# eivindeb/fixed-wing-gym

Measured on AMD Instinct MI355X. Metric: env-steps/sec, higher is better.
Workload: dtype f32

## Files before the change

fixed-wing-gym_amd/csrc/fwgym.hip:

```cpp
#include <math.h>
#include <stdio.h>
#include <string.h>
#include <string>
#include <vector>
#include "fwgym_env.h"
#include "fwgym_actor.h"
#include "fwgym_learner.h"

__device__ __forceinline__ float wave_sum(float v) { return wave_sum64(v); }

struct SpecWords { unsigned w[sizeof(DevCfg) / 4]; };
static_assert(sizeof(SpecWords) == sizeof(DevCfg), "DevCfg must be made of 32-bit members only");
#if defined(FWG_SPECS_FILE)
#include FWG_SPECS_FILE
#elif defined(FWG_WITH_SPECS)
#include "generated/specs.inc"
#else
#define FWG_SPEC_LIST(X)
#endif
#ifndef FWG_SHAPE_LIST
#define FWG_SHAPE_LIST(X)
#endif
#define FWG_SHAPE_BASE FWG_INSTANCE_SHAPE
#define FWG_DEFINE_SPEC(i) static constexpr DevCfg kSpec##i = __builtin_bit_cast(DevCfg, kSpecWords##i);
FWG_SPEC_LIST(FWG_DEFINE_SPEC)
template <int SPEC> struct SpecCfg {
    static constexpr int obs_dim = 16;
    static constexpr bool rollout_ok = false;
    static constexpr bool one_rk4_step = false;
    static __device__ __forceinline__ const DevCfg& get(const DevCfg* cp) { return *cp; }
};
#define FWG_SPEC_GETTER(i)                                                                                \
    template <> struct SpecCfg<i> {                                                                       \
        static constexpr int obs_dim = kSpec##i.obs_dim;                                                  \
        static constexpr bool one_rk4_step = kSpec##i.nsub == 1;                                          \
         \
        static constexpr bool rollout_ok = kSpec##i.obs_log == 0 && kSpec##i.obs_dim <= 64;               \
        static __device__ __forceinline__ const DevCfg& get(const DevCfg*) { return kSpec##i; }           \
    };
FWG_SPEC_LIST(FWG_SPEC_GETTER)
#define FWG_SHAPE_OBJECT(i) static constexpr DevCfg kShape##i = as_shape(kSpec##i);
FWG_SHAPE_LIST(FWG_SHAPE_OBJECT)
#define FWG_SHAPE_GETTER(i)                                                                               \
    template <> struct SpecCfg<FWG_SHAPE_BASE + i> {                                                      \
        static constexpr int obs_dim = kSpec##i.obs_dim;                                                  \
        static constexpr bool one_rk4_step = kSpec##i.nsub == 1;                                          \
        static constexpr bool rollout_ok = false;    \
        static __device__ __forceinline__ const DevCfg& get(const DevCfg*) { return kShape##i; }          \
    };
FWG_SHAPE_LIST(FWG_SHAPE_GETTER)

template <int SPEC> struct KernelTypes {
    typedef LdsTable Tab;
    typedef LdsTable Obs;
    static constexpr bool generic = true;
    static __device__ __forceinline__ Tab tab(float* lds, const LdsMap& M, int lane) { return Tab{lds + M.tab + lane}; }
    static __device__ __forceinline__ Obs obs(float* lds, const LdsMap& M, int lane) { return Obs{lds + M.obs + lane}; }
};
#define FWG_SPEC_TYPES(i)                                                                                     \
    template <> struct KernelTypes<i> {                      \
        typedef RegTable<FWG_TAB_ROWS> Tab;                                                                   \
        typedef RegTable<kSpec##i.obs_dim> Obs;                                                               \
        static constexpr bool generic = false;                                                                \
        static __device__ __forceinline__ Tab tab(float*, const LdsMap&, int) { return Tab(); }               \
        static __device__ __forceinline__ Obs obs(float*, const LdsMap&, int) { return Obs(); }               \
    };
FWG_SPEC_LIST(FWG_SPEC_TYPES)
#define FWG_SHAPE_TYPES(i) template <> struct KernelTypes<FWG_SHAPE_BASE + i> : KernelTypes<i> {};
FWG_SHAPE_LIST(FWG_SHAPE_TYPES)

struct NoHeadStats { static constexpr bool enabled = false; const float* mean = nullptr; float ret_mean = 0.f; unsigned ctr = 0u; };
struct HeadStats { static constexpr bool enabled = true; const float* mean; float ret_mean; unsigned ctr; };
template <class OB, class HS = NoHeadStats>
__device__ __forceinline__ void step_moments(const DevCfg& c, const KArgs& A, const OB& ob, float reward, bool done, bool valid,
                                             int lane, long e, int sub, float ret_prev, const HS& hs = HS()) {
#ifndef FWG_ABL_NO_ACC
    const int D = c.obs_dim;
    float dr = 0.f;
    if (valid) {
        const float r = ret_prev * A.acc_gamma + reward;
        A.acc_ret[e] = done ? 0.f : r;
        dr = r - (HS::enabled ? hs.ret_mean : *(FWG_KCONST(float)*)A.acc_ret_mean);
    }
    const unsigned ctr = HS::enabled ? hs.ctr : *(FWG_KCONST(unsigned)*)A.acc_ctr;
    unsigned long long* acc = A.acc + (size_t)(ctr % FWG_ACC_SETS) * FWG_ACC_SHARDS * A.acc_cols;
    FWG_KCONST(float)* mean_k = (FWG_KCONST(float)*)A.acc_mean;
    const float one = valid ? 1.f : 0.f;
#pragma unroll
    for (int chunk = 0; chunk < (2 * FWG_MAX_OBS * FWG_MAX_ROWS + 4 + 31) / 32; ++chunk) {
        if (32 * chunk < 2 * D + 4) {
            float dev[16], mean[16];
            if (HS::enabled) {
                float4 q[5];
#pragma unroll
                for (int g = 0; g < 5; ++g) {
                    const int k0 = 16 * chunk - 4 + 4 * g;
                    q[g] = make_float4(0.f, 0.f, 0.f, 0.f);
                    if (k0 >= 0 && k0 < D && k0 + 3 < FWG_ACT_MAX_OBS) q[g] = *reinterpret_cast<const float4*>(hs.mean + k0);
                }
#pragma unroll
                for (int g = 0; g < 5; ++g) { q[g].x = rounded(q[g].x); q[g].y = rounded(q[g].y); q[g].z = rounded(q[g].z); q[g].w = rounded(q[g].w); }
#pragma unroll
                for (int j = 0; j < 16; ++j) {
                    const float4 g = q[(j + 2) >> 2];
                    mean[j] = ((j + 2) & 3) == 0 ? g.x : ((j + 2) & 3) == 1 ? g.y : ((j + 2) & 3) == 2 ? g.z : g.w;
                }
            }
#pragma unroll
            for (int j = 0; j < 16; ++j) {
                const int k = 16 * chunk - 2 + j;
                dev[j] = 0.f;
                if (k >= 0 && k < D && k < FWG_MAX_OBS * FWG_MAX_ROWS) {
                    const float m = HS::enabled ? mean[j] : mean_k[k];
                    dev[j] = valid ? ob.get(k) - m : 0.f;
                }
            }
            float v[32];
#pragma unroll
            for (int i = 0; i < 32; ++i) {
                const int col = 32 * chunk + i;
                v[i] = col == 0 ? dr : col == 1 ? dr * dr : (col == 2 || col == 3) ? one : ((i & 1) == 0 ? dev[i >> 1] : dev[i >> 1] * dev[i >> 1]);
            }
#ifdef FWG_ABL_NO_TOTALS
            acc_flush(acc, A.acc_cols, sub & (FWG_ACC_SHARDS - 1), chunk, lane, v[0] + v[7] + v[13] + v[27]);
#else
            acc_flush(acc, A.acc_cols, sub & (FWG_ACC_SHARDS - 1), chunk, lane, wave_totals32(v, lane));
#endif
        }
    }
#endif
}

struct PartnerActuators {
    static constexpr bool enabled = true;
    const float* p;
    __device__ __forceinline__ void fetch_half(float (&a_half)[5]) const {
        const float4 q = fwg_msg_take(p, FWG_TAG_ACTS);
        a_half[0] = q.x; a_half[1] = q.y; a_half[2] = q.z;
    }
    __device__ __forceinline__ void fetch_full(float (&a_full)[5]) const {
        const float4 q2 = fwg_msg_take(p + 8, FWG_TAG_ACTS);
        const float4 q1 = reinterpret_cast<const float4*>(p)[1];
        a_full[0] = q1.x; a_full[1] = q1.y; a_full[2] = q1.z; a_full[3] = q1.w; a_full[4] = q2.x;
    }
};
struct StageStamps {
    const KArgs& A;
    __device__ __forceinline__ void operator()(int st) const { FWG_TL(A, 26 + st); }
};
struct HandToGym {
    static constexpr bool enabled = true;
    float* h;
    const KArgs* A;
    __device__ __forceinline__ void state(const float (&yy)[NY], const float (&ea)[5]) const {
        float4* h4 = reinterpret_cast<float4*>(h);
        h4[0] = make_float4(yy[4], yy[5], yy[6], yy[7]);
        h4[1] = make_float4(yy[8], yy[9], yy[10], yy[11]);
        h4[2] = make_float4(yy[12], yy[13], yy[14], yy[15]);
        h4[3] = make_float4(ea[0], ea[1], ea[2], ea[3]);
        fwg_msg_put(h + 16, ea[4], 0.f, 0.f, FWG_TAG_STATE);
        FWG_TL(*A, 30);
    }
    __device__ __forceinline__ void result(float Va, float alpha, float beta, int fail) const {
        fwg_msg_put(h + 20, Va, alpha, beta, FWG_TAG_RESULT | (unsigned)fail);
        FWG_TL(*A, 31);
    }
};

template <bool TURB, int SPEC, int ROLE, class HS = NoHeadStats>
__device__ __forceinline__ void step_wave(const DevCfg* __restrict__ cp, const DynCfg* __restrict__ dp, const KArgs& A0, float* lds, int sub,
                                          const float* act_lds = nullptr, const HS& hs = HS()) {
    typedef KernelTypes<SPEC> KT;
    constexpr bool PHYS = ROLE != 2, GYM = ROLE != 1, SPLIT = ROLE != 0;
    const DevCfg& c = SpecCfg<SPEC>::get(cp);
    KArgs A_ = resolve_slots(c, A0);
    if constexpr (!HS::enabled && SPLIT && GYM) {
        if (A_.acc != nullptr) {
            const char* st = reinterpret_cast<const char*>(fwg_fresh_scalar_view(A_.acc_mean)) - offsetof(ActorStats, mean);
            A_.acc_mean = reinterpret_cast<const float*>(st + offsetof(ActorStats, mean));
            A_.acc_ret_mean = reinterpret_cast<const float*>(st + offsetof(ActorStats, ret_mean));
            A_.acc_ctr = reinterpret_cast<const unsigned*>(st + offsetof(ActorStats, act_counter));
        }
    }
    const KArgs& A = A_;
    if (PHYS && A0.slots_out != nullptr && sub == 0 && (threadIdx.x & (FWG_WAVE - 1)) == 0)
        *A0.slots_out = next_slots(c.obs_step, c.obs_log, c.obs_length, c.L.window, c.L.lag_depth, c.streak_req, load_slots(A0.slots_in));
#ifdef FWG_ABL_EMPTY
    return;
#endif
    DynCfgK& dc = *(DynCfgK*)dp;
    FWG_TL(A, 0);
    const int lane = threadIdx.x & (FWG_WAVE - 1);
    const long env0 = (long)sub * FWG_WAVE;
    const bool valid = env0 + lane < A.N;
    const long e = valid ? env0 + lane : A.N - 1;
    const LdsMap M = lds_map(c.obs_dim, c.n_obs, c.L.window, c.use_cmd_ring, KT::generic, c.obs_log, SPLIT);
    const fwg_layout& L = c.L;
    const int W = L.window;
    typename KT::Tab T = KT::tab(lds, M, lane);
    typename KT::Obs ob = KT::obs(lds, M, lane);
    float* aring = lds + M.aring + lane * 4;
    float* cring = lds + M.cring + lane * 4;
    float* hand = lds + M.stage + lane * FWG_HAND_WORDS;
    float* tailm = lds + M.stage + FWG_WAVE * FWG_HAND_WORDS + lane * FWG_TAIL_WORDS;
    float* acts = lds + M.stage + FWG_WAVE * (FWG_HAND_WORDS + FWG_TAIL_WORDS) + lane * FWG_ACT_WORDS;
    float* mark = lds + M.flag;
    constexpr bool ext_act = SPLIT && SpecCfg<SPEC>::one_rk4_step;

    constexpr bool gym_waits = SPLIT && GYM && ext_act;
    float raw[3] = {0.f, 0.f, 0.f};
    if (!gym_waits) {
#pragma unroll
        for (int i = 0; i < 3; ++i) raw[i] = HS::enabled ? act_lds[lane * 4 + i] : A.actions[e * 3 + i];
    }
    Env E;
    float4 act_q3 = make_float4(0.f, 0.f, 0.f, 0.f), act_q4 = act_q3;
    if (PHYS) load_sim<TURB>(c, A.S, A.N, e, E);
    if (!gym_waits) load_cold(c, A.S, A.N, e, E);
    Aero la;
    if (PHYS && (KT::generic || c.model_n > 0)) {
        if (c.model_n > 0) load_aero(c, A.S, A.N, e, la); else aero_from_cfg(c, la);
    }
    const bool tail_rows = SPLIT && !HS::enabled && c.obs_log > 0 && c.obs_length > 1 && A.acc == nullptr;
    const bool pre_install = SPLIT && !HS::enabled && c.auto_reset && (c.obs_log > 0 || !c.obs_noise) &&
                             V(c).steps_max > (c.obs_length - 1) * c.obs_step + 1 &&
                             A.acc == nullptr && !c.has_int_obs;
    const bool partner_rows = pre_install && c.obs_log > 0 && c.obs_length > 1;

    if (SPLIT) {
        if (PHYS) {
            fwg_msg_put(hand + 16, 0.f, 0.f, 0.f, 0u);
            fwg_msg_put(hand + 20, 0.f, 0.f, 0.f, 0u);
            fwg_msg_put(hand + 24, 0.f, 0.f, 0.f, 0u);
            fwg_msg_put(hand + 8, 0.f, 0.f, 0.f, 0u);
            if (lane == 0) FWG_FLAG_RAISE(mark, 0);
        } else {
            fwg_msg_put(acts, 0.f, 0.f, 0.f, 0u);
            fwg_msg_put(acts + 8, 0.f, 0.f, 0.f, 0u);
            fwg_msg_put(tailm, 0.f, 0.f, 0.f, 0u);
        }
#ifndef FWG_ABL_NO_ENTRY_BARRIER
        FWG_BLOCK_SYNC_LDS();
#endif
    }
    if (SPLIT) FWG_SETPRIO(PHYS ? FWG_PRIO_PHYS_STAGES : FWG_PRIO_GYM_EARLY);
    if (SPLIT && ext_act) {
        if (PHYS) {
            float4* h4 = reinterpret_cast<float4*>(hand);
            h4[0] = make_float4(E.y[13], E.y[14], E.y[15], E.y[16]);
            h4[1] = make_float4(E.y[17], raw[0], raw[1], raw[2]);
            fwg_msg_put(hand + 8, 0.f, 0.f, 0.f, FWG_TAG_RAW);
        } else {
            fwg_msg_take(hand + 8, FWG_TAG_RAW);
            const float4 q0 = reinterpret_cast<const float4*>(hand)[0], q1 = reinterpret_cast<const float4*>(hand)[1];
            act_q3 = make_float4(0.f, q0.x, q0.y, q0.z); act_q4 = make_float4(q0.w, q1.x, 0.f, 0.f);
            raw[0] = q1.y; raw[1] = q1.z; raw[2] = q1.w;
            load_cold(c, A.S, A.N, e, E);
        }
    }
    float ret_prev = 0.f;
    float wa[FWG_MAX_WINDOW][3], wc[FWG_MAX_WINDOW][3];
    float4 int_old = make_float4(0.f, 0.f, 0.f, 0.f);
    float4 sum_prev = make_float4(0.f, 0.f, 0.f, 0.f);
    auto late_rows = [&]() {
#ifndef FWG_ABL_NO_LATE_ROWS
        if (SPLIT) load_gym(c, A.S, A.N, e, E, A.bit_goal, 2);
#endif
        if (c.metrics) {
            int slot = A.slot_end - 1; slot += (slot < 0) ? FWG_END_RING : 0;
            sum_prev = CGROUP(A.S, A.N, (L.end_ring >> 2) + slot, e);
        }
        if (c.int_window) {
            int slot = A.slot_end - (c.int_window + 1); slot += (slot < 0) ? FWG_END_RING : 0;
            int_old = CGROUP(A.S, A.N, (L.end_ring >> 2) + slot, e);
        }
    };
    if (GYM) {
#ifdef FWG_ABL_NO_LATE_ROWS
        constexpr bool LATE = false;
#else
        constexpr bool LATE = SPLIT;
#endif
        load_gym(c, A.S, A.N, e, E, A.bit_goal, LATE ? 1 : 3);
        if (!LATE) late_rows();
        if (A.acc != nullptr && valid) ret_prev = A.acc_ret[e];
        if (SPLIT) {
#pragma unroll
            for (int k = 1; k < FWG_MAX_WINDOW; ++k) {
                if (k < W) {
                    int slot = A.slot_act - k; slot += (slot < 0) ? W : 0;
                    const float4 qa = CGROUP(A.S, A.N, (L.act_ring >> 2) + slot, e);
                    wa[k][0] = qa.x; wa[k][1] = qa.y; wa[k][2] = qa.z;
                    if (c.use_cmd_ring) {
                        const float4 qc = CGROUP(A.S, A.N, (L.cmd_ring >> 2) + slot, e);
                        wc[k][0] = qc.x; wc[k][1] = qc.y; wc[k][2] = qc.z;
                    }
                }
            }
        }
    }
    if (GYM && valid) GROUP(A.S, A.N, (L.act_ring >> 2) + A.slot_act, e) = make_float4(raw[0], raw[1], raw[2], 0.f);

    float cmd[3];
#pragma unroll
    for (int i = 0; i < 3; ++i) {
// ... 1819 lines not shown

static size_t actor_lds_bytes(int nk1, int parts) {
    return (size_t)(actor_weight_floats(nk1, parts) + actor_scratch_floats()) * sizeof(float);
}

static ActorArgs actor_args(const fwg_actor* a) {
    ActorArgs A;
    memset(&A, 0, sizeof(A));
    A.ret = a->d_ret; A.stats = a->d_stats; A.frags = a->d_frags; A.bias = a->d_bias; A.log_std = a->d_log_std;
    A.acc = a->d_acc; A.acc_cols = a->acc_cols;
    A.N = (long)a->n_envs; A.env_base = (long)a->env_base;
    A.D = a->D; A.nk1 = a->nk1; A.act_dim = a->act_dim; A.parity = a->parity; A.training = a->training;
    A.gamma = a->gamma; A.clip_obs = a->clip_obs; A.clip_rew = a->clip_rew; A.eps = a->eps;
    A.seed_lo = (unsigned)(a->seed & 0xFFFFFFFFull); A.seed_hi = (unsigned)(a->seed >> 32);
#ifdef FWG_TIMELINE
    A.trace = a->trace;
#endif
    if (a->log_env != nullptr) {
        const fwg_handle* h = a->log_env;
        A.obs_n = h->h.n_obs;
        A.obs_win = host_slots(h, h->gstep - 1).log_win;
        A.obs_slots = h->graph_mode ? h->d_slots + ((h->gstep - 1) & 1) : nullptr;
    }
    return A;
}

static void observer_args(fwg_handle* h, KArgs* A) {
    fwg_actor* a = h->observer;
    if (!a) return;
    A->acc = a->d_acc;
    A->acc_ctr = &a->d_stats[a->parity].act_counter;
    A->acc_mean = a->d_stats[a->parity].mean; A->acc_ret_mean = &a->d_stats[a->parity].ret_mean;
    A->acc_ret = a->d_ret; A->acc_gamma = a->gamma; A->acc_cols = a->acc_cols;
}

extern "C" {

int fwg_attach_observer(fwg_handle* h, fwg_actor* a) {
    if (!h) return fail_with(FWG_ERR_INVALID, "fwg_attach_observer: null env handle");
    if (a && h->h.obs_log > 0)
        return fail_with(FWG_ERR_INVALID, "fwg_attach_observer: row-log observations keep the lagged rows out of the step kernel; use fwg_actor_observe");
    if (a && (a->n_envs != h->n_envs || a->D != h->h.obs_dim || a->device != h->device))
        return fail_with(FWG_ERR_INVALID, "fwg_attach_observer: the head was created for another batch size / observation size / device");
    h->observer = a;
    h->rollout_lds_granted = 0;
    if (a && h->spec >= 0 && h->split && launch_rollout(h, a, KArgs(), ActorArgs(), nullptr, true) == 0)
        h->rollout_lds_granted = launch_rollout(h, a, KArgs(), ActorArgs(), nullptr, false, true) == 0 ? 1 : 0;
    return FWG_OK;
}

#ifdef FWG_TIMELINE
int fwg_debug_set_actor_trace(fwg_actor* a, long long* trace_dev) { if (!a) return FWG_ERR_INVALID; a->trace = trace_dev; return FWG_OK; }
#endif
int fwg_actor_set_obs_log(fwg_actor* a, const fwg_handle* env) {
    if (!a) return fail_with(FWG_ERR_INVALID, "fwg_actor_set_obs_log: null actor");
    if (env != nullptr) {
        if (env->h.obs_log <= 0) return fail_with(FWG_ERR_INVALID, "fwg_actor_set_obs_log: the env writes the dense observation batch");
        if (env->n_envs != a->n_envs || env->h.obs_dim != a->D || env->device != a->device || (env->h.n_obs & 3))
            return fail_with(FWG_ERR_INVALID, "fwg_actor_set_obs_log: batch size / observation size / device mismatch (n_obs must be a multiple of 4)");
    }
    a->log_env = env;
    return FWG_OK;
}

int fwg_actor_create(int device, int64_t n_envs, int obs_dim, int act_dim, float gamma, float clip_obs, float clip_reward,
                     float epsilon, fwg_actor** out) {
    if (!out) return fail_with(FWG_ERR_INVALID, "fwg_actor_create: null argument");
    if (n_envs < 1) return fail_with(FWG_ERR_INVALID, "fwg_actor_create: n_envs < 1");
    if (obs_dim < 1 || obs_dim > FWG_ACT_MAX_OBS) return fail_with(FWG_ERR_INVALID, "fwg_actor_create: obs_dim must be in [1, 64]");
    if (act_dim < 1 || act_dim > FWG_ACT_MAX_ACT) return fail_with(FWG_ERR_INVALID, "fwg_actor_create: act_dim must be in [1, 4]");
    HIP_TRY(hipSetDevice(device));
    fwg_actor* a = new fwg_actor();
    memset(a, 0, sizeof(*a));
    a->device = device; a->n_envs = n_envs; a->D = obs_dim; a->act_dim = act_dim; a->nk1 = (obs_dim + 15) / 16;
    a->gamma = gamma; a->clip_obs = clip_obs; a->clip_rew = clip_reward; a->eps = epsilon;
    a->training = 1; a->precise = 1;
    const size_t nfrag = (size_t)2 * 2 * actor_frags(a->nk1) * 64;
    HIP_TRY(hipMalloc((void**)&a->d_stats, 2 * sizeof(ActorStats)));
    a->acc_cols = acc_cols_for(obs_dim);
    const size_t acc_bytes = (size_t)FWG_ACC_SETS * FWG_ACC_SHARDS * a->acc_cols * sizeof(unsigned long long);
    HIP_TRY(hipMalloc((void**)&a->d_acc, acc_bytes));
    HIP_TRY(hipMemset(a->d_acc, 0, acc_bytes));
    HIP_TRY(hipMalloc((void**)&a->d_frags, nfrag * sizeof(frag_t)));
    HIP_TRY(hipMalloc((void**)&a->d_bias, 2 * FWG_ACT_BIAS_FLOATS * sizeof(float)));
    HIP_TRY(hipMemset(a->d_bias, 0, 2 * FWG_ACT_BIAS_FLOATS * sizeof(float)));
    HIP_TRY(hipMalloc((void**)&a->d_log_std, FWG_ACT_MAX_ACT * sizeof(float)));
    HIP_TRY(hipMalloc((void**)&a->d_ret, (size_t)n_envs * sizeof(float)));
    HIP_TRY(hipMemset(a->d_frags, 0, nfrag * sizeof(frag_t)));
    HIP_TRY(hipMemset(a->d_log_std, 0, FWG_ACT_MAX_ACT * sizeof(float)));
    HIP_TRY(hipMemset(a->d_ret, 0, (size_t)n_envs * sizeof(float)));
    ActorStats s[2];
    memset(s, 0, sizeof(s));
    for (int p = 0; p < 2; ++p) {
        for (int f = 0; f < FWG_ACT_MAX_OBS; ++f) s[p].var[f] = 1.f;
        s[p].count = 1e-4f; s[p].ret_var = 1.f; s[p].ret_count = 1e-4f;
    }
    HIP_TRY(hipMemcpy(a->d_stats, s, sizeof(s), hipMemcpyHostToDevice));
    a->lds_act[0] = actor_lds_bytes(a->nk1, 1);
    a->lds_act[1] = actor_lds_bytes(a->nk1, 2);
    {
        const void* k1[4] = {(const void*)k_actor_act<1, 1>, (const void*)k_actor_act<1, 2>, (const void*)k_actor_act<1, 3>, (const void*)k_actor_act<1, 4>};
        const void* k3[4] = {(const void*)k_actor_act<3, 1>, (const void*)k_actor_act<3, 2>, (const void*)k_actor_act<3, 3>, (const void*)k_actor_act<3, 4>};
        HIP_TRY(hipFuncSetAttribute(k1[a->nk1 - 1], hipFuncAttributeMaxDynamicSharedMemorySize, (int)a->lds_act[0]));
        HIP_TRY(hipFuncSetAttribute(k3[a->nk1 - 1], hipFuncAttributeMaxDynamicSharedMemorySize, (int)a->lds_act[1]));
    }
    *out = a;
    return FWG_OK;
}

void fwg_actor_destroy(fwg_actor* a) {
    if (!a) return;
    (void)hipFree(a->d_stats); (void)hipFree(a->d_acc); (void)hipFree(a->d_frags); (void)hipFree(a->d_bias); (void)hipFree(a->d_log_std); (void)hipFree(a->d_ret);
    delete a;
}

int fwg_actor_set_weights(fwg_actor* a, const fwg_actor_weights* w) {
    if (!a || !w) return fail_with(FWG_ERR_INVALID, "fwg_actor_set_weights: null argument");
    const float* const need[] = {w->pi_w0, w->pi_b0, w->pi_w1, w->pi_b1, w->pi_w2, w->pi_b2,
                                 w->vf_w0, w->vf_b0, w->vf_w1, w->vf_b1, w->vf_w2, w->vf_b2, w->log_std};
    for (const float* p : need) if (!p) return fail_with(FWG_ERR_INVALID, "fwg_actor_set_weights: null weight array");
    HIP_TRY(hipSetDevice(a->device));
    std::vector<unsigned> all;
    std::vector<float> biases;
    for (int net = 0; net < 2; ++net) {
        std::vector<unsigned> hi, lo;
        const float* w0 = net ? w->vf_w0 : w->pi_w0; const float* b0 = net ? w->vf_b0 : w->pi_b0;
        const float* w1 = net ? w->vf_w1 : w->pi_w1; const float* b1 = net ? w->vf_b1 : w->pi_b1;
        const float* w2 = net ? w->vf_w2 : w->pi_w2; const float* b2 = net ? w->vf_b2 : w->pi_b2;
        const int out = net ? 1 : a->act_dim;
        actor_pack_layer(hi, lo, w0, 64, a->D, 2, a->nk1, false, FWG_ACT_PRESCALE);
        actor_pack_layer(hi, lo, w1, 64, 64, 2, 4, true, FWG_ACT_PRESCALE);
        actor_pack_layer(hi, lo, w2, out, 64, 1, 4, true, 1.f);
        all.insert(all.end(), hi.begin(), hi.end());
        all.insert(all.end(), lo.begin(), lo.end());
        actor_pack_bias(biases, b0, b1, b2, out);
    }
    HIP_TRY(hipMemcpy(a->d_bias, biases.data(), biases.size() * sizeof(float), hipMemcpyHostToDevice));
    const size_t want = (size_t)2 * 2 * actor_frags(a->nk1) * 64 * 4;
    if (all.size() != want) return fail_with(FWG_ERR_INVALID, "fwg_actor_set_weights: internal packing size mismatch");
    HIP_TRY(hipMemcpy(a->d_frags, all.data(), all.size() * sizeof(unsigned), hipMemcpyHostToDevice));
    float ls[FWG_ACT_MAX_ACT] = {0.f, 0.f, 0.f, 0.f};
    for (int i = 0; i < a->act_dim; ++i) ls[i] = w->log_std[i];
    HIP_TRY(hipMemcpy(a->d_log_std, ls, sizeof(ls), hipMemcpyHostToDevice));
    return FWG_OK;
}

int fwg_actor_set_stats(fwg_actor* a, const fwg_actor_stats* s, void* stream) {
    if (!a || !s) return fail_with(FWG_ERR_INVALID, "fwg_actor_set_stats: null argument");
    HIP_TRY(hipSetDevice(a->device));
    HIP_TRY(hipStreamSynchronize((hipStream_t)stream));
    ActorStats cur;
    HIP_TRY(hipMemcpy(&cur, a->d_stats + a->parity, sizeof(cur), hipMemcpyDeviceToHost));
    memcpy(cur.mean, s->obs_mean, sizeof(cur.mean));
    memcpy(cur.var, s->obs_var, sizeof(cur.var));
    cur.count = s->obs_count; cur.ret_mean = s->ret_mean; cur.ret_var = s->ret_var; cur.ret_count = s->ret_count;
    HIP_TRY(hipMemcpy(a->d_stats + a->parity, &cur, sizeof(cur), hipMemcpyHostToDevice));
    return FWG_OK;
}

int fwg_actor_get_stats(fwg_actor* a, fwg_actor_stats* s, void* stream) {
    if (!a || !s) return fail_with(FWG_ERR_INVALID, "fwg_actor_get_stats: null argument");
    HIP_TRY(hipSetDevice(a->device));
    HIP_TRY(hipStreamSynchronize((hipStream_t)stream));
    ActorStats cur;
    HIP_TRY(hipMemcpy(&cur, a->d_stats + a->parity, sizeof(cur), hipMemcpyDeviceToHost));
    memcpy(s->obs_mean, cur.mean, sizeof(cur.mean));
    memcpy(s->obs_var, cur.var, sizeof(cur.var));
    s->obs_count = cur.count; s->ret_mean = cur.ret_mean; s->ret_var = cur.ret_var; s->ret_count = cur.ret_count;
    return FWG_OK;
}

int fwg_actor_configure(fwg_actor* a, int training, int precise) {
    if (!a) return fail_with(FWG_ERR_INVALID, "fwg_actor_configure: null handle");
    a->training = training ? 1 : 0;
    a->precise = precise ? 1 : 0;
    return FWG_OK;
}

int fwg_actor_seed(fwg_actor* a, uint64_t seed, int64_t env_id_base) {
    if (!a) return fail_with(FWG_ERR_INVALID, "fwg_actor_seed: null handle");
    a->seed = seed; a->env_base = env_id_base;
    return FWG_OK;
}

int fwg_actor_observe(fwg_actor* a, const float* obs, const float* reward, const uint8_t* done, void* stream) {
    if (!a) return fail_with(FWG_ERR_INVALID, "fwg_actor_observe: null handle");
    if (!obs && !reward) return FWG_OK;
    HIP_TRY(hipSetDevice(a->device));
    ActorArgs A = actor_args(a);
    A.obs = obs; A.rew = reward; A.done = done;
    const dim3 grid((unsigned)((a->n_envs + FWG_ACT_BLOCK - 1) / FWG_ACT_BLOCK)), block(FWG_ACT_BLOCK);
    hipLaunchKernelGGL(k_actor_stats, grid, block, 0, (hipStream_t)stream, A);
    HIP_TRY(hipGetLastError());
    return FWG_OK;
}

int fwg_actor_act(fwg_actor* a, const float* obs, const float* reward, const uint8_t* done, float* norm_obs_out,
                  float* action_out, float* value_out, float* logp_out, float* norm_reward_out, uint8_t* done_out,
                  int deterministic, void* stream) {
    if (!a || !obs) return fail_with(FWG_ERR_INVALID, "fwg_actor_act: null argument");
    HIP_TRY(hipSetDevice(a->device));
    ActorArgs A = actor_args(a);
    A.obs = obs; A.rew = reward; A.done = done;
    A.norm_obs = norm_obs_out; A.action = action_out; A.value = value_out; A.logp = logp_out; A.norm_rew = norm_reward_out;
    A.done_out = done_out; A.deterministic = deterministic ? 1 : 0;
    const dim3 grid((unsigned)((a->n_envs + FWG_ACT_ENVS - 1) / FWG_ACT_ENVS)), block(64 * FWG_ACT_WAVES);
    hipStream_t st = (hipStream_t)stream;
#define FWG_ACT_LAUNCH(NK)                                                                                \
    case NK:                                                                                              \
        if (a->precise) hipLaunchKernelGGL((k_actor_act<3, NK>), grid, block, a->lds_act[1], st, A);     \
        else hipLaunchKernelGGL((k_actor_act<1, NK>), grid, block, a->lds_act[0], st, A);                \
        break;
    switch (a->nk1) { FWG_ACT_LAUNCH(1) FWG_ACT_LAUNCH(2) FWG_ACT_LAUNCH(3) FWG_ACT_LAUNCH(4) default: break; }
#undef FWG_ACT_LAUNCH
    HIP_TRY(hipGetLastError());
    a->parity ^= 1;
    return FWG_OK;
}

}
template <bool TURB, int SPEC>
static int launch_rollout_one(fwg_handle* h, fwg_actor* a, const KArgs& A, const ActorArgs& AA, hipStream_t stream, bool grant) {
    if constexpr (SPEC >= 0) {
        if constexpr (SpecCfg<SPEC>::rollout_ok) {
            if (grant) {
                const size_t b3 = (size_t)rollout_lds_floats(h->h, 3) * sizeof(float), b1 = (size_t)rollout_lds_floats(h->h, 1) * sizeof(float);
                if (b3 > 160 * 1024 || b1 > 160 * 1024) return 1;
                if (hipFuncSetAttribute((const void*)k_rollout<TURB, SPEC, 3>, hipFuncAttributeMaxDynamicSharedMemorySize, (int)b3) != hipSuccess) return 1;
                if (hipFuncSetAttribute((const void*)k_rollout<TURB, SPEC, 1>, hipFuncAttributeMaxDynamicSharedMemorySize, (int)b1) != hipSuccess) return 1;
                return 0;
            }
            const int hsplit = a->precise ? 3 : 1;
            const size_t bytes = (size_t)rollout_lds_floats(h->h, hsplit) * sizeof(float);
            if (bytes > 160 * 1024 || !h->rollout_lds_granted) return 1;
            const dim3 grid((unsigned)((h->n_envs + FWG_RO_ENVS - 1) / FWG_RO_ENVS)), block(2 * FWG_RO_ENVS);
            if (a->precise) hipLaunchKernelGGL((k_rollout<TURB, SPEC, 3>), grid, block, bytes, stream, h->d_cfg, h->d_dyn, A, AA);
            else hipLaunchKernelGGL((k_rollout<TURB, SPEC, 1>), grid, block, bytes, stream, h->d_cfg, h->d_dyn, A, AA);
            return 0;
        }
    }
    return 1;
}
static int launch_rollout(fwg_handle* h, fwg_actor* a, const KArgs& A, const ActorArgs& AA, hipStream_t stream, bool probe, bool grant) {
    switch (h->spec) {
#define FWG_SPEC_RO(i) \
    case i: if (probe) return (SpecCfg<i>::rollout_ok && (size_t)rollout_lds_floats(kSpec##i, 3) * sizeof(float) <= 160 * 1024) ? 0 : 1; \
            return launch_rollout_one<(kSpec##i.turbulence != 0), i>(h, a, A, AA, stream, grant);
        FWG_SPEC_LIST(FWG_SPEC_RO)
#undef FWG_SPEC_RO
        default: break;
    }
    return 1;
}

extern "C" {

int fwg_rollout_available(const fwg_handle* h, const fwg_actor* a) {
    if (!h || !a || h->observer != a || h->spec < 0 || !h->split || h->h.obs_log > 0) return 0;
    if (h->h.model_n > 0 || h->h.randomize_scaling) return 0;
    if (a->act_dim != 3 || a->log_env != nullptr) return 0;
    if (!h->rollout_lds_granted) return 0;
    return launch_rollout(const_cast<fwg_handle*>(h), const_cast<fwg_actor*>(a), KArgs(), ActorArgs(), nullptr, true) == 0 ? 1 : 0;
}

int fwg_rollout_step(fwg_handle* h, fwg_actor* a, float* norm_obs_out, float* action_out, float* value_out, float* logp_out,
                     float* norm_reward_out, uint8_t* done_prev_out, float* obs_io, float* reward_io, uint8_t* done_io,
                     uint8_t* term_code_out, float* terminal_obs_out, float* metrics_out, int deterministic, void* stream) {
    if (!h || !a || !obs_io || !reward_io || !done_io || !term_code_out) return fail_with(FWG_ERR_INVALID, "fwg_rollout_step: null argument");
    if (!fwg_rollout_available(h, a))
        return fail_with(FWG_ERR_INVALID, "fwg_rollout_step: needs a build-time specialised configuration with the dense observation batch "
                                          "and this head attached (fwg_attach_observer); use fwg_step + fwg_actor_act otherwise");
    HIP_TRY(hipSetDevice(a->device));
    ActorArgs AA = actor_args(a);
    AA.obs = obs_io; AA.rew = reward_io; AA.done = done_io;
    AA.norm_obs = norm_obs_out; AA.action = action_out; AA.value = value_out; AA.logp = logp_out; AA.norm_rew = norm_reward_out;
    AA.done_out = done_prev_out; AA.deterministic = deterministic ? 1 : 0;
    KArgs A;
    base_args(h, &A);
    A.actions = nullptr; A.obs = obs_io; A.rew = reward_io; A.done = done_io; A.term = term_code_out;
    A.term_obs = terminal_obs_out; A.metrics = metrics_out; A.tgt_out = nullptr;
    h->last_metrics_out = metrics_out;
    fill_slots(h, h->gstep, &A);
    if (h->graph_mode) { A.slots_in = h->d_slots + (h->gstep & 1); A.slots_out = h->d_slots + ((h->gstep + 1) & 1); }
    a->parity ^= 1;
    observer_args(h, &A);
#ifdef FWG_TIMELINE
    A.trace = h->trace;
#endif
    if (launch_rollout(h, a, A, AA, (hipStream_t)stream, false) != 0) {
        a->parity ^= 1;
        return fail_with(FWG_ERR_INVALID, "fwg_rollout_step: no fused launch for this configuration");
    }
    HIP_TRY(hipGetLastError());
    h->gstep += 1;
    return FWG_OK;
}

}

struct fwg_learner {
    fwg_actor* head;
    PpoLayout L;
    float* d_slab;
    float* d_grad;
};

static PpoBatch ppo_batch(const fwg_ppo_batch* b) {
    PpoBatch B;
    B.obs = b->obs; B.act = b->actions; B.val = b->values; B.logp = b->logp; B.adv = b->adv; B.ret = b->returns;
    return B;
}
static bool ppo_batch_ok(const fwg_ppo_batch* b) {
    return b && b->obs && b->actions && b->values && b->logp && b->adv && b->returns;
}
static int ppo_launch_grad(fwg_learner* L, const fwg_ppo_batch* b, const int64_t* idx, int64_t mb, const float* moments,
                           const float* params, const fwg_ppo_hparams* hp, float* grad_out, hipStream_t st) {
    PpoGradArgs G;
    G.B = ppo_batch(b); G.idx = (const long long*)idx; G.mb = (long)mb; G.mom = moments; G.params = params;
    G.hp = (const PpoHparams*)hp; G.slab = L->d_slab; G.L = L->L;
    G.ntiles = (long)((mb + FWG_PPO_ROWS - 1) / FWG_PPO_ROWS);
    const unsigned nb = (unsigned)(G.ntiles < FWG_PPO_MAX_BLOCKS ? G.ntiles : FWG_PPO_MAX_BLOCKS);
    hipLaunchKernelGGL(k_ppo_grad, dim3(nb), dim3(FWG_PPO_THREADS), (size_t)ppo_grad_lds_floats() * sizeof(float), st, G);
    HIP_TRY(hipGetLastError());
    const int n = L->L.P + FWG_PPO_NSTAT;
    hipLaunchKernelGGL(k_ppo_reduce, dim3((unsigned)((n + FWG_PPO_THREADS - 1) / FWG_PPO_THREADS)), dim3(FWG_PPO_THREADS), 0, st,
                       (const float*)L->d_slab, (int)nb, L->L, (const PpoHparams*)hp, grad_out);
    HIP_TRY(hipGetLastError());
    return FWG_OK;
}

extern "C" {

int fwg_learner_create(fwg_actor* head, fwg_learner** out) {
    if (!head || !out) return fail_with(FWG_ERR_INVALID, "fwg_learner_create: null argument");
    HIP_TRY(hipSetDevice(head->device));
    fwg_learner* L = new fwg_learner();
    L->head = head;
    L->L = ppo_layout(head->D, head->act_dim);
    HIP_TRY(hipMalloc((void**)&L->d_slab, (size_t)FWG_PPO_MAX_BLOCKS * L->L.SW * sizeof(float)));
    HIP_TRY(hipMalloc((void**)&L->d_grad, (size_t)(L->L.P + FWG_PPO_NSTAT) * sizeof(float)));
    HIP_TRY(hipMemset(L->d_slab, 0, (size_t)FWG_PPO_MAX_BLOCKS * L->L.SW * sizeof(float)));
    HIP_TRY(hipMemset(L->d_grad, 0, (size_t)(L->L.P + FWG_PPO_NSTAT) * sizeof(float)));
    HIP_TRY(hipFuncSetAttribute((const void*)k_ppo_grad, hipFuncAttributeMaxDynamicSharedMemorySize, (int)(ppo_grad_lds_floats() * sizeof(float))));
    *out = L;
    return FWG_OK;
}

void fwg_learner_destroy(fwg_learner* L) {
    if (!L) return;
    (void)hipFree(L->d_slab); (void)hipFree(L->d_grad);
    delete L;
}

int64_t fwg_learner_num_params(const fwg_learner* L) { return L ? (int64_t)L->L.P : -1; }

int fwg_ppo_moments(fwg_learner* L, const float* adv, const int64_t* perm, int64_t mb, int n_minibatches, float* moments, void* stream) {
    if (!L || !adv || !perm || !moments) return fail_with(FWG_ERR_INVALID, "fwg_ppo_moments: null argument");
    if (mb < 1 || n_minibatches < 1) return fail_with(FWG_ERR_INVALID, "fwg_ppo_moments: mb and n_minibatches must be positive");
    hipLaunchKernelGGL(k_ppo_moments, dim3((unsigned)n_minibatches), dim3(FWG_PPO_THREADS), FWG_PPO_THREADS * sizeof(double), (hipStream_t)stream,
                       adv, (const long long*)perm, (long)mb, moments);
    HIP_TRY(hipGetLastError());
    return FWG_OK;
}

int fwg_ppo_grad(fwg_learner* L, const fwg_ppo_batch* b, const int64_t* idx, int64_t mb, const float* moments, const float* params,
                 const fwg_ppo_hparams* hp, float* grad_out, void* stream) {
    if (!L || !ppo_batch_ok(b) || !idx || !moments || !params || !hp || !grad_out) return fail_with(FWG_ERR_INVALID, "fwg_ppo_grad: null argument");
    if (mb < 1) return fail_with(FWG_ERR_INVALID, "fwg_ppo_grad: mb must be positive");
    return ppo_launch_grad(L, b, idx, mb, moments, params, hp, grad_out, (hipStream_t)stream);
}

int fwg_ppo_apply(fwg_learner* L, const float* grad, int64_t mb, const fwg_ppo_hparams* hp, float* params, float* adam_m, float* adam_v,
                  int32_t* step, float* stats_acc, void* stream) {
    if (!L || !grad || !hp || !params || !adam_m || !adam_v || !step || !stats_acc) return fail_with(FWG_ERR_INVALID, "fwg_ppo_apply: null argument");
    if (mb < 1) return fail_with(FWG_ERR_INVALID, "fwg_ppo_apply: mb must be positive");
    hipLaunchKernelGGL(k_ppo_apply, dim3(1), dim3(FWG_PPO_APPLY_THREADS), FWG_PPO_APPLY_THREADS * sizeof(float), (hipStream_t)stream,
                       grad, (long)mb, L->L, (const PpoHparams*)hp, params, adam_m, adam_v, (int*)step, stats_acc);
    HIP_TRY(hipGetLastError());
    return FWG_OK;
}

int fwg_ppo_step(fwg_learner* L, const fwg_ppo_batch* b, const int64_t* idx, int64_t mb, const float* moments, const fwg_ppo_hparams* hp,
                 float* params, float* adam_m, float* adam_v, int32_t* step, float* stats_acc, void* stream) {
    if (!L || !ppo_batch_ok(b) || !idx || !moments || !hp || !params || !adam_m || !adam_v || !step || !stats_acc)
        return fail_with(FWG_ERR_INVALID, "fwg_ppo_step: null argument");
    if (mb < 1) return fail_with(FWG_ERR_INVALID, "fwg_ppo_step: mb must be positive");
    const int rc = ppo_launch_grad(L, b, idx, mb, moments, params, hp, L->d_grad, (hipStream_t)stream);
    if (rc != FWG_OK) return rc;
    return fwg_ppo_apply(L, L->d_grad, mb, hp, params, adam_m, adam_v, step, stats_acc, stream);
}

int fwg_actor_pack(fwg_learner* L, const float* params, void* stream) {
    if (!L || !params) return fail_with(FWG_ERR_INVALID, "fwg_actor_pack: null argument");
    const fwg_actor* a = L->head;
    const int n = 2 * actor_frags(a->nk1) * 64 + 2 * FWG_ACT_BIAS_FLOATS + FWG_ACT_MAX_ACT;
    hipLaunchKernelGGL(k_actor_pack, dim3((unsigned)((n + 255) / 256)), dim3(256), 0, (hipStream_t)stream, params, L->L, a->nk1,
                       a->d_frags, a->d_bias, a->d_log_std);
    HIP_TRY(hipGetLastError());
    return FWG_OK;
}

}
```

fixed-wing-gym_amd/csrc/fwgym_learner.h:

```cpp
#pragma once
#include "fwgym_actor.h"

#define FWG_PPO_ROWS 64
#define FWG_PPO_THREADS 256
#define FWG_PPO_MAX_BLOCKS 256
#define FWG_PPO_LS 65
#define FWG_PPO_NSTAT 4
#define FWG_PPO_APPLY_THREADS 256

struct PpoHparams { double lr, cliprange, ent_coef, vf_coef, max_grad_norm, beta1, beta2, eps; };
struct PpoLayout { int D, A, P, SW; int ls, w1[2], b1[2], w2[2], b2[2], w3[2], b3[2]; };
struct PpoBatch { const float *obs, *act, *val, *logp, *adv, *ret; };

__host__ __device__ inline PpoLayout ppo_layout(int D, int A) {
    PpoLayout L;
    L.D = D; L.A = A;
    int o = 0;
    L.ls = o; o += A;
    for (int net = 0; net < 2; ++net) {
        const int nout = net ? 1 : A;
        L.w1[net] = o; o += 64 * D;
        L.b1[net] = o; o += 64;
        L.w2[net] = o; o += 64 * 64;
        L.b2[net] = o; o += 64;
        L.w3[net] = o; o += nout * 64;
        L.b3[net] = o; o += nout;
    }
    L.P = o;
    L.SW = (o + FWG_PPO_NSTAT + 3) & ~3;
    return L;
}

__device__ __forceinline__ float ppo_tanh(float z) { return tanh_prescaled(FWG_ACT_PRESCALE * z); }

__device__ __forceinline__ void ppo_mma_tile(f32x16& acc, const float* A, int sam, int sak, int m0, int ml, const float* B, int sbk,
                                             int sbn, int n0, int nl, int K, int kl, int l) {
    const int i = l & 31, half = l >> 5;
    const bool mok = m0 + i < ml, nok = n0 + i < nl;
    for (int k0 = 0; k0 < K; k0 += 16) {
        float a[8], b[8];
#pragma unroll
        for (int t = 0; t < 8; ++t) {
            const int k = k0 + 8 * half + t;
            a[t] = (mok && k < kl) ? A[(m0 + i) * sam + k * sak] : 0.f;
            b[t] = (nok && k < kl) ? B[k * sbk + (n0 + i) * sbn] : 0.f;
        }
        frag_t ah, al, bh, bl;
        split8(a, ah, al);
        split8(b, bh, bl);
        acc = mma3<3>(ah, al, bh, bl, acc);
    }
}
__device__ __forceinline__ int ppo_acc_row(int r, int half) { return (r & 3) + 8 * (r >> 2) + 4 * half; }

__global__ __launch_bounds__(FWG_PPO_THREADS) void k_ppo_moments(const float* __restrict__ adv, const long long* __restrict__ perm,
                                                                 long mb, float* __restrict__ mom) {
    extern __shared__ __attribute__((aligned(16))) float lds[];
    double* red = reinterpret_cast<double*>(lds);
    const int tid = threadIdx.x;
    const long long* idx = perm + (long)blockIdx.x * mb;
    double s = 0.0;
    for (long i = tid; i < mb; i += FWG_PPO_THREADS) s += (double)adv[idx[i]];
    red[tid] = s;
    __syncthreads();
    for (int w = FWG_PPO_THREADS / 2; w > 0; w >>= 1) {
        if (tid < w) red[tid] += red[tid + w];
        __syncthreads();
    }
    const double mean = red[0] / (double)mb;
    __syncthreads();
    double q = 0.0;
    for (long i = tid; i < mb; i += FWG_PPO_THREADS) {
        const double d = (double)adv[idx[i]] - mean;
        q += d * d;
    }
    red[tid] = q;
    __syncthreads();
    for (int w = FWG_PPO_THREADS / 2; w > 0; w >>= 1) {
        if (tid < w) red[tid] += red[tid + w];
        __syncthreads();
    }
    if (tid == 0) {
        mom[2 * blockIdx.x] = (float)mean;
        mom[2 * blockIdx.x + 1] = (float)sqrt(red[0] / (double)mb) + 1e-8f;
    }
}

struct PpoGradArgs {
    PpoBatch B;
    const long long* idx;
    long mb;
    long ntiles;
    const float* mom;
    const float* params;
    const PpoHparams* hp;
    float* slab;
    PpoLayout L;
};
__host__ __device__ inline int ppo_grad_lds_floats() { return 5 * FWG_PPO_ROWS * FWG_PPO_LS + 4 * FWG_PPO_ROWS + 8 * FWG_PPO_ROWS + 8 * FWG_PPO_ROWS; }

__global__ __launch_bounds__(FWG_PPO_THREADS) void k_ppo_grad(const PpoGradArgs G) {
    extern __shared__ __attribute__((aligned(16))) float lds[];
    constexpr int LS = FWG_PPO_LS;
    const int tid = threadIdx.x, l = tid & 63, wv = tid >> 6, half = l >> 5;
    const PpoLayout& L = G.L;
    const int D = L.D, A = L.A, nk1 = (D + 15) / 16;
    float* Xs = lds;
    float* H1 = Xs + FWG_PPO_ROWS * LS;
    float* H2 = H1 + FWG_PPO_ROWS * LS;
    float* Gb = H2 + FWG_PPO_ROWS * LS;
    float* Tb = Gb + FWG_PPO_ROWS * LS;
    float* dO = Tb + FWG_PPO_ROWS * LS;
    float* rowf = dO + 4 * FWG_PPO_ROWS;
    float* red = rowf + 8 * FWG_PPO_ROWS;
    const PpoHparams hp = *G.hp;
    const float adv_mean = G.mom[0], adv_std = G.mom[1];
    const float inv_mb = 1.f / (float)G.mb, clip = (float)hp.cliprange, vf_coef = (float)hp.vf_coef;
    const float* P = G.params;
    const long t0 = (long)blockIdx.x * G.ntiles / gridDim.x, t1 = (long)(blockIdx.x + 1) * G.ntiles / gridDim.x;
    const int tm0 = 32 * (wv & 1), tn0 = 32 * (wv >> 1);
    const int vo = tid >> 6, vk = tid & 63;
    f32x16 gw1[2], gw2[2];
#pragma unroll
    for (int r = 0; r < 16; ++r) { gw1[0][r] = 0.f; gw1[1][r] = 0.f; gw2[0][r] = 0.f; gw2[1][r] = 0.f; }
    float gw3[2] = {0.f, 0.f}, gb3[2] = {0.f, 0.f}, gb2[2] = {0.f, 0.f}, gb1[2] = {0.f, 0.f};
    float gls[FWG_ACT_MAX_ACT] = {0.f, 0.f, 0.f, 0.f}, st[FWG_PPO_NSTAT] = {0.f, 0.f, 0.f, 0.f};
    for (long t = t0; t < t1; ++t) {
        const long r0 = t * FWG_PPO_ROWS;
        const int nrows = (int)(G.mb - r0 < FWG_PPO_ROWS ? G.mb - r0 : FWG_PPO_ROWS);
        {
            const int r = tid >> 2, q = tid & 3;
            const bool ok = r < nrows;
            const long long row = ok ? G.idx[r0 + r] : 0;
            for (int f = 16 * q; f < 16 * q + 16; ++f) Xs[r * LS + f] = (ok && f < D) ? G.B.obs[row * D + f] : 0.f;
            if (q == 0) {
#pragma unroll
                for (int a = 0; a < FWG_ACT_MAX_ACT; ++a) rowf[r * 8 + a] = (ok && a < A) ? G.B.act[row * A + a] : 0.f;
                rowf[r * 8 + 4] = ok ? G.B.val[row] : 0.f;
                rowf[r * 8 + 5] = ok ? G.B.logp[row] : 0.f;
                rowf[r * 8 + 6] = ok ? (G.B.adv[row] - adv_mean) / adv_std : 0.f;
                rowf[r * 8 + 7] = ok ? G.B.ret[row] : 0.f;
            }
        }
        __syncthreads();
#pragma unroll
        for (int net = 0; net < 2; ++net) {
            const int nout = net ? 1 : A;
            const float *W1 = P + L.w1[net], *b1 = P + L.b1[net], *W2 = P + L.w2[net], *b2 = P + L.b2[net];
            const float *W3 = P + L.w3[net], *b3 = P + L.b3[net];
            {
                f32x16 acc = {0.f};
                ppo_mma_tile(acc, Xs, LS, 1, tm0, 64, W1, 1, D, tn0, 64, 16 * nk1, D, l);
                const int n = tn0 + (l & 31);
                const float bn = b1[n];
#pragma unroll
                for (int r = 0; r < 16; ++r) H1[(tm0 + ppo_acc_row(r, half)) * LS + n] = ppo_tanh(acc[r] + bn);
            }
            __syncthreads();
            {
                f32x16 acc = {0.f};
                ppo_mma_tile(acc, H1, LS, 1, tm0, 64, W2, 1, 64, tn0, 64, 64, 64, l);
                const int n = tn0 + (l & 31);
                const float bn = b2[n];
#pragma unroll
                for (int r = 0; r < 16; ++r) H2[(tm0 + ppo_acc_row(r, half)) * LS + n] = ppo_tanh(acc[r] + bn);
            }
            __syncthreads();
            if (vo < nout) {
                float o = b3[vo];
                for (int k = 0; k < 64; ++k) o += H2[vk * LS + k] * W3[vo * 64 + k];
                dO[vk * 4 + vo] = o;
            }
            __syncthreads();
            if (tid < FWG_PPO_ROWS) {
                const int r = tid;
                const bool ok = r < nrows;
                const float* rf = rowf + r * 8;
                if (net == 0) {
                    float nl = 0.9189385332046727f * (float)A, z[FWG_ACT_MAX_ACT], is[FWG_ACT_MAX_ACT];
#pragma unroll
                    for (int a = 0; a < FWG_ACT_MAX_ACT; ++a) {
                        z[a] = 0.f; is[a] = 0.f;
                        if (a < A) {
                            const float s = P[L.ls + a];
                            is[a] = expf(-s);
                            z[a] = (rf[a] - dO[r * 4 + a]) * is[a];
                            nl += 0.5f * z[a] * z[a] + s;
                        }
                    }
                    const float ratio = expf(-rf[5] - nl), adv = rf[6];
                    const float rc = fminf(fmaxf(ratio, 1.f - clip), 1.f + clip);
                    const float p1 = -adv * ratio, p2 = -adv * rc;
                    const float g1 = -adv, g2 = (ratio >= 1.f - clip && ratio <= 1.f + clip) ? -adv : 0.f;
                    const float dr = p1 > p2 ? g1 : (p1 < p2 ? g2 : 0.5f * (g1 + g2));
                    const float gn = ok ? -ratio * dr * inv_mb : 0.f;
#pragma unroll
                    for (int a = 0; a < FWG_ACT_MAX_ACT; ++a) {
                        dO[r * 4 + a] = a < A ? -gn * z[a] * is[a] : 0.f;
                        gls[a] += a < A ? gn * (1.f - z[a] * z[a]) : 0.f;
                    }
                    if (ok) {
                        const float kl = nl + rf[5];
                        st[0] += fmaxf(p1, p2);
                        st[2] += 0.5f * kl * kl;
                        st[3] += fabsf(ratio - 1.f) > clip ? 1.f : 0.f;
                    }
                } else {
                    const float v = dO[r * 4], ov = rf[4], R = rf[7], d = v - ov;
                    const float vc = ov + fminf(fmaxf(d, -clip), clip);
                    const float l1 = (v - R) * (v - R), l2 = (vc - R) * (vc - R);
                    const float g1 = 2.f * (v - R), g2 = (d >= -clip && d <= clip) ? 2.f * (vc - R) : 0.f;
                    const float dv = l1 > l2 ? g1 : (l1 < l2 ? g2 : 0.5f * (g1 + g2));
                    dO[r * 4] = ok ? vf_coef * 0.5f * dv * inv_mb : 0.f;
                    if (ok) st[1] += 0.5f * fmaxf(l1, l2);
                }
            }
            __syncthreads();
            if (vo < nout) {
                float s = 0.f, sb = 0.f;
                for (int r = 0; r < FWG_PPO_ROWS; ++r) { s += dO[r * 4 + vo] * H2[r * LS + vk]; sb += dO[r * 4 + vo]; }
                gw3[net] += s;
                if (vk == 0) gb3[net] += sb;
            }
            for (int j = 0; j < FWG_PPO_ROWS * 64 / FWG_PPO_THREADS; ++j) {
                const int e = tid + FWG_PPO_THREADS * j, r = e >> 6, k = e & 63;
                float s = 0.f;
                for (int o = 0; o < nout; ++o) s += dO[r * 4 + o] * W3[o * 64 + k];
                const float h = H2[r * LS + k];
                Gb[r * LS + k] = s * (1.f - h * h);
            }
            __syncthreads();
            {
                f32x16 acc = {0.f};
                ppo_mma_tile(acc, Gb, LS, 1, tm0, 64, W2, 64, 1, tn0, 64, 64, 64, l);
                const int n = tn0 + (l & 31);
#pragma unroll
                for (int r = 0; r < 16; ++r) {
                    const int m = tm0 + ppo_acc_row(r, half);
                    const float h = H1[m * LS + n];
                    Tb[m * LS + n] = acc[r] * (1.f - h * h);
                }
                ppo_mma_tile(gw2[net], Gb, 1, LS, tm0, 64, H1, LS, 1, tn0, 64, 64, 64, l);
                if (tid < 64) {
                    float s = 0.f;
                    for (int r = 0; r < FWG_PPO_ROWS; ++r) s += Gb[r * LS + tid];
                    gb2[net] += s;
                }
            }
            __syncthreads();
            if (tn0 < D) ppo_mma_tile(gw1[net], Tb, 1, LS, tm0, 64, Xs, LS, 1, tn0, D, 64, 64, l);
            if (tid < 64) {
                float s = 0.f;
                for (int r = 0; r < FWG_PPO_ROWS; ++r) s += Tb[r * LS + tid];
                gb1[net] += s;
            }
            __syncthreads();
        }
    }
    float* S = G.slab + (size_t)blockIdx.x * L.SW;
#pragma unroll
    for (int net = 0; net < 2; ++net) {
        const int nout = net ? 1 : A;
        const int n = tn0 + (l & 31);
#pragma unroll
        for (int r = 0; r < 16; ++r) {
            const int m = tm0 + ppo_acc_row(r, half);
            if (n < D) S[L.w1[net] + m * D + n] = gw1[net][r];
            S[L.w2[net] + m * 64 + n] = gw2[net][r];
        }
        if (vo < nout) {
            S[L.w3[net] + vo * 64 + vk] = gw3[net];
            if (vk == 0) S[L.b3[net] + vo] = gb3[net];
        }
        if (tid < 64) { S[L.b1[net] + tid] = gb1[net]; S[L.b2[net] + tid] = gb2[net]; }
    }
    if (tid < FWG_PPO_ROWS) {
#pragma unroll
        for (int a = 0; a < 4; ++a) { red[tid * 8 + a] = gls[a]; red[tid * 8 + 4 + a] = st[a]; }
    }
    __syncthreads();
    if (tid < 8) {
        float s = 0.f;
        for (int r = 0; r < FWG_PPO_ROWS; ++r) s += red[r * 8 + tid];
        if (tid < A) S[L.ls + tid] = s;
        else if (tid >= 4) S[L.P + tid - 4] = s;
    }
}

__global__ __launch_bounds__(FWG_PPO_THREADS) void k_ppo_reduce(const float* __restrict__ slab, int nslab, const PpoLayout L,
                                                                const PpoHparams* __restrict__ hp, float* __restrict__ grad) {
    const int j = blockIdx.x * FWG_PPO_THREADS + threadIdx.x;
    if (j >= L.P + FWG_PPO_NSTAT) return;
    float s = 0.f;
    for (int b = 0; b < nslab; ++b) s += slab[(size_t)b * L.SW + j];
    if (j >= L.ls && j < L.ls + L.A) s -= (float)hp->ent_coef;
    grad[j] = s;
}

__global__ __launch_bounds__(FWG_PPO_APPLY_THREADS) void k_ppo_apply(const float* __restrict__ grad, long mb, const PpoLayout L,
                                                                     const PpoHparams* __restrict__ hp, float* __restrict__ params,
                                                                     float* __restrict__ m1, float* __restrict__ m2, int* __restrict__ step,
                                                                     float* __restrict__ acc) {
    extern __shared__ __attribute__((aligned(16))) float lds[];
    const int tid = threadIdx.x;
    float ent = 0.f;
    if (tid == 0)
        for (int a = 0; a < L.A; ++a) ent += params[L.ls + a] + 1.4189385332046727f;
    float ss = 0.f;
    for (int j = tid; j < L.P; j += FWG_PPO_APPLY_THREADS) ss += grad[j] * grad[j];
    lds[tid] = ss;
    __syncthreads();
    for (int w = FWG_PPO_APPLY_THREADS / 2; w > 0; w >>= 1) {
        if (tid < w) lds[tid] += lds[tid + w];
        __syncthreads();
    }
    const PpoHparams h = *hp;
    const float norm = sqrtf(lds[0]);
    const float coef = fminf((float)h.max_grad_norm / (norm + 1e-6f), 1.f);
    const int t = *step + 1;
    const double bc1 = 1.0 - pow(h.beta1, (double)t), bc2 = 1.0 - pow(h.beta2, (double)t);
    const float step_size = (float)(h.lr / bc1), bc2_sqrt = (float)sqrt(bc2);
    const float b2 = (float)h.beta2, w1 = (float)(1.0 - h.beta1), w2 = (float)(1.0 - h.beta2), eps = (float)h.eps;
    for (int j = tid; j < L.P; j += FWG_PPO_APPLY_THREADS) {
        const float g = grad[j] * coef;
        float m = m1[j], v = m2[j];
        m = m + w1 * (g - m);
        v = v * b2 + w2 * (g * g);
        m1[j] = m; m2[j] = v;
        params[j] -= step_size * (m / (sqrtf(v) / bc2_sqrt + eps));
    }
    __syncthreads();
    if (tid == 0) {
        const float inv = 1.f / (float)mb;
        *step = t;
        acc[0] += grad[L.P] * inv;
        acc[1] += grad[L.P + 1] * inv;
        acc[2] += ent;
        acc[3] += grad[L.P + 2] * inv;
        acc[4] += grad[L.P + 3] * inv;
    }
}

__global__ __launch_bounds__(256) void k_actor_pack(const float* __restrict__ params, const PpoLayout L, int nk1, frag_t* __restrict__ frags,
                                                    float* __restrict__ bias, float* __restrict__ log_std) {
    const int nfw = actor_frags(nk1);
    const int nfrag_thr = 2 * nfw * 64;
    const int g = blockIdx.x * 256 + threadIdx.x;
    if (g < nfrag_thr) {
        const int net = g / (nfw * 64), f = (g / 64) % nfw, l = g & 63, half = l >> 5;
        const int nout = net ? 1 : L.A;
        const float* W;
        int out, in, it, kk;
        bool chained;
        float scale;
        if (f < 2 * nk1) { W = params + L.w1[net]; out = 64; in = L.D; it = f / nk1; kk = f % nk1; chained = false; scale = FWG_ACT_PRESCALE; }
        else if (f < 2 * nk1 + 8) { W = params + L.w2[net]; out = 64; in = 64; it = (f - 2 * nk1) / 4; kk = (f - 2 * nk1) % 4; chained = true; scale = FWG_ACT_PRESCALE; }
        else { W = params + L.w3[net]; out = nout; in = 64; it = 0; kk = f - 2 * nk1 - 8; chained = true; scale = 1.f; }
        const int i = 32 * it + (l & 31);
        unsigned wh[4] = {0u, 0u, 0u, 0u}, wl[4] = {0u, 0u, 0u, 0u};
#pragma unroll
        for (int t = 0; t < 8; ++t) {
            const int k = chained ? k_chained(kk, half, t) : k_input(kk, half, t);
            const float v = (i < out && k < in) ? scale * W[i * in + k] : 0.f;
            const unsigned h16 = bf16_rne(v), l16 = bf16_rne(v - bf16_to_f32(h16));
            wh[t >> 1] |= h16 << (16 * (t & 1));
            wl[t >> 1] |= l16 << (16 * (t & 1));
        }
        frags[((net * 2 + 0) * nfw + f) * 64 + l] = frag_t{wh[0], wh[1], wh[2], wh[3]};
        frags[((net * 2 + 1) * nfw + f) * 64 + l] = frag_t{wl[0], wl[1], wl[2], wl[3]};
        return;
    }
    const int j = g - nfrag_thr;
    if (j < 2 * FWG_ACT_BIAS_FLOATS) {
        const int net = j / FWG_ACT_BIAS_FLOATS, c = j % FWG_ACT_BIAS_FLOATS;
        const int nout = net ? 1 : L.A;
        float v;
        if (c < 64) v = FWG_ACT_PRESCALE * params[L.b1[net] + c];
        else if (c < 128) v = FWG_ACT_PRESCALE * params[L.b2[net] + c - 64];
        else v = c - 128 < nout ? params[L.b3[net] + c - 128] : 0.f;
        bias[j] = v;
    } else if (j < 2 * FWG_ACT_BIAS_FLOATS + FWG_ACT_MAX_ACT) {
        const int a = j - 2 * FWG_ACT_BIAS_FLOATS;
        log_std[a] = a < L.A ? params[L.ls + a] : 0.f;
    }
}
```

fixed-wing-gym_amd/gym_fixed_wing/ppo.py:

```python
import math

import numpy as np
import torch
from torch import nn

from . import _native as nat
from .rollout import FusedRollout, MlpPolicy

PPO2_DEFAULTS = dict(gamma=0.99, n_steps=128, ent_coef=0.01, learning_rate=2.5e-4, vf_coef=0.5, max_grad_norm=0.5, lam=0.95,
                     nminibatches=4, noptepochs=4, cliprange=0.2)


STAT_KEYS = ("pg_loss", "vf_loss", "entropy", "approx_kl", "clip_frac")


def sb_init_(policy):
    for net, out_gain in ((policy.pi, 0.01), (policy.vf, 1.0)):
        lin = [m for m in net if isinstance(m, nn.Linear)]
        for i, m in enumerate(lin):
            nn.init.orthogonal_(m.weight, gain=out_gain if i == len(lin) - 1 else math.sqrt(2.0))
            nn.init.zeros_(m.bias)
    with torch.no_grad():
        policy.log_std.zero_()
    return policy


def gae(lib, mem, rewards, values, dones, last_value, gamma, lam, adv_out=None, ret_out=None):
    import ctypes
    T, N = int(rewards.shape[0]), int(rewards.shape[1])
    adv_out = mem.zeros((T, N)) if adv_out is None else adv_out
    ret_out = mem.zeros((T, N)) if ret_out is None else ret_out
    nat.check(lib, lib.fwg_gae(T, N, mem.ptr(rewards), mem.ptr(values), mem.ptr(dones), mem.ptr(last_value),
                               ctypes.c_float(gamma), ctypes.c_float(lam), mem.ptr(adv_out), mem.ptr(ret_out), mem.stream()))
    return adv_out, ret_out


def ppo_loss(policy, obs, actions, old_values, old_logp, adv, returns, cliprange, ent_coef, vf_coef):
    adv = (adv - adv.mean()) / (adv.std(unbiased=False) + 1e-8)
    mean = policy.pi(obs)
    value = policy.vf(obs).squeeze(-1)
    log_std = policy.log_std
    neglogp = 0.5 * (((actions - mean) / log_std.exp()) ** 2).sum(dim=-1) + 0.5 * math.log(2.0 * math.pi) * actions.shape[-1] + log_std.sum()
    ratio = torch.exp(-old_logp - neglogp)
    pg_loss = torch.max(-adv * ratio, -adv * torch.clamp(ratio, 1.0 - cliprange, 1.0 + cliprange)).mean()
    v_clipped = old_values + torch.clamp(value - old_values, -cliprange, cliprange)
    vf_loss = 0.5 * torch.max((value - returns) ** 2, (v_clipped - returns) ** 2).mean()
    entropy = (log_std + 0.5 * math.log(2.0 * math.pi * math.e)).sum()
    loss = pg_loss - ent_coef * entropy + vf_coef * vf_loss
    with torch.no_grad():
        stats = {"pg_loss": pg_loss.detach(), "vf_loss": vf_loss.detach(), "entropy": entropy.detach(),
                 "approx_kl": 0.5 * ((neglogp + old_logp) ** 2).mean(), "clip_frac": ((ratio - 1.0).abs() > cliprange).float().mean()}
    return loss, stats


class PPO(object):

    def __init__(self, vec, policy=None, seed=0, fused=None, graph=True, curriculum=None, group=None, precise=True,
                 graph_update=True, update="torch", **kw):
        from .actor import DeviceActor
        hp = dict(PPO2_DEFAULTS)
        unknown = set(kw) - set(hp)
        if unknown:
            raise TypeError("unknown PPO hyper-parameters: {}".format(sorted(unknown)))
        hp.update(kw)
        if update not in ("torch", "hip"):
            raise ValueError("update must be 'torch' or 'hip', not {!r}".format(update))
        self.update_path = update
        self.hp, self.vec, self.group = hp, vec, group
        self.n_steps = int(hp["n_steps"])
        self._torch_dev = getattr(vec._mem, "device", torch.device("cpu"))
        torch.manual_seed(seed)
        self.policy = (sb_init_(MlpPolicy(vec.obs_dim)) if policy is None else policy).to(self._torch_dev)
        self.actor = DeviceActor.for_env(vec, seed=seed, gamma=hp["gamma"], precise=precise)
        self.actor.load_policy(self.policy)
        self._rollout_kw = dict(graph=bool(graph) and self._torch_dev.type == "cuda", fused=fused)
        self.rollout = FusedRollout(vec, self.actor, self.n_steps, **self._rollout_kw)
        self._spec_at_capture = vec.spec_index
        on_gpu = self._torch_dev.type == "cuda"
        if update == "hip":
            from .learner import HipLearner
            self.opt, self._lr = None, hp["learning_rate"]
            self.learner = HipLearner(vec._lib, self.actor, self.policy, self._torch_dev, graph=bool(graph_update) and on_gpu)
        else:
            self.opt = torch.optim.Adam(self.policy.parameters(), lr=hp["learning_rate"], eps=1e-5, **({"capturable": True, "fused": True} if on_gpu else {}))
        self._graph_update, self._step_graph = bool(graph_update) and on_gpu, None
        self.curriculum = curriculum
        m, N, T = vec._mem, vec.num_envs, self.n_steps
        self.adv, self.ret = m.zeros((T, N)), m.zeros((T, N))
        self.num_timesteps, self.updates = 0, 0
        self.history = []
        self._gen = torch.Generator(device=self._torch_dev)
        self._gen.manual_seed(seed + 1)
        self._world = 1
        if torch.distributed.is_available() and torch.distributed.is_initialized():
            self._world = torch.distributed.get_world_size(group)
            for p in self.policy.parameters():
                torch.distributed.broadcast(p.data, src=0, group=group)
            self.actor.load_policy(self.policy)

    def _t(self, x):
        return torch.as_tensor(x) if not isinstance(x, torch.Tensor) else x

    def collect(self):
        buf = self.rollout.run()
        gae(self.vec._lib, self.vec._mem, buf["rewards"], buf["values"], buf["dones"], self.rollout.last_value,
            self.hp["gamma"], self.hp["lam"], self.adv, self.ret)
        T, N = self.n_steps, self.vec.num_envs
        self.num_timesteps += T * N * self._world
        flat = lambda x, *s: self._t(x).reshape((T * N,) + s)
        return {"obs": flat(buf["obs"], self.vec.obs_dim), "actions": flat(buf["actions"], 3), "values": flat(buf["values"]),
                "logp": flat(buf["logp"]), "adv": flat(self.adv), "returns": flat(self.ret)}

    def _minibatch_step(self, mbatch, cliprange):
        hp = self.hp
        loss, stats = ppo_loss(self.policy, mbatch["obs"], mbatch["actions"], mbatch["values"], mbatch["logp"], mbatch["adv"],
                               mbatch["returns"], cliprange, hp["ent_coef"], hp["vf_coef"])
        self.opt.zero_grad(set_to_none=False)
        loss.backward()
        if self._world > 1:
            flat = torch.cat([p.grad.reshape(-1) for p in self.policy.parameters()])
            torch.distributed.all_reduce(flat, group=self.group)
            flat /= self._world
            o = 0
            for p in self.policy.parameters():
                p.grad.copy_(flat[o:o + p.numel()].view_as(p))
                o += p.numel()
        nn.utils.clip_grad_norm_(self.policy.parameters(), hp["max_grad_norm"])
        self.opt.step()
        return torch.stack([stats[k] for k in STAT_KEYS])

    def _capture_step(self, batch, mb, cliprange):
        dev = self._torch_dev
        g = {"idx": torch.zeros(mb, dtype=torch.long, device=dev), "acc": torch.zeros(len(STAT_KEYS), device=dev), "src": batch,
             "key": (tuple(int(batch[k].data_ptr()) for k in sorted(batch)), mb, float(cliprange))}
        snap_p = [p.detach().clone() for p in self.policy.parameters()]
        snap_o = [{k: v.clone() for k, v in st.items() if isinstance(v, torch.Tensor)} for st in self.opt.state.values()]

        D = batch["obs"].shape[1]
        g["packed"] = torch.empty((batch["obs"].shape[0], D + 7), device=dev)
        g["pack"] = lambda: torch.cat([batch["obs"], batch["actions"], batch["values"][:, None], batch["logp"][:, None],
                                       batch["adv"][:, None], batch["returns"][:, None]], dim=1, out=g["packed"])
        g["pack"]()

        def body():
            m = g["packed"].index_select(0, g["idx"])
            mbatch = {"obs": m[:, :D], "actions": m[:, D:D + 3], "values": m[:, D + 3], "logp": m[:, D + 4], "adv": m[:, D + 5],
                      "returns": m[:, D + 6]}
            g["acc"].add_(self._minibatch_step(mbatch, cliprange))

        g["idx"].copy_(torch.arange(mb, device=dev))
        side = torch.cuda.Stream(device=dev)
        side.wait_stream(torch.cuda.current_stream(dev))
        with torch.cuda.stream(side):
            for _ in range(3):
                body()
        torch.cuda.current_stream(dev).wait_stream(side)
        torch.cuda.synchronize(dev)
        had_state = len(snap_o) > 0
        with torch.no_grad():
            for p, q in zip(self.policy.parameters(), snap_p):
                p.copy_(q)
            for i, st in enumerate(self.opt.state.values()):
                for k, v in st.items():
                    if isinstance(v, torch.Tensor):
                        v.copy_(snap_o[i][k]) if had_state else v.zero_()
        g["graph"] = torch.cuda.CUDAGraph()
        with torch.cuda.graph(g["graph"]):
            body()
        g["acc"].zero_()
        return g

    def _update_hip(self, batch, lr, cliprange):
        hp = self.hp
        n = batch["obs"].shape[0]
        nmb = int(hp["nminibatches"])
        if lr is not None:
            self._lr = lr
        perms = [torch.randperm(n, device=self._torch_dev, generator=self._gen) for _ in range(int(hp["noptepochs"]))]
        stats = self.learner.update(batch, perms, n // nmb, nmb, self._lr, hp["cliprange"] if cliprange is None else cliprange,
                                    hp["ent_coef"], hp["vf_coef"], hp["max_grad_norm"], world=self._world, group=self.group)
        self.updates += 1
        return stats

    def update(self, batch, lr=None, cliprange=None):
        if self.update_path == "hip":
            return self._update_hip(batch, lr, cliprange)
        hp = self.hp
        n = batch["obs"].shape[0]
        mb = n // int(hp["nminibatches"])
        cliprange = hp["cliprange"] if cliprange is None else cliprange
        if lr is not None:
            for g in self.opt.param_groups:
                g["lr"] = lr
        graphed = self._graph_update and self._world == 1 and lr is None
        if graphed:
            key = (tuple(int(batch[k].data_ptr()) for k in sorted(batch)), mb, float(cliprange))
            if self._step_graph is None or self._step_graph["key"] != key:
                self._step_graph = self._capture_step(batch, mb, cliprange)
            sg = self._step_graph
            sg["pack"]()
            sg["acc"].zero_()
        acc = torch.zeros(len(STAT_KEYS), device=self._torch_dev)
        for _ in range(int(hp["noptepochs"])):
            perm = torch.randperm(n, device=self._torch_dev, generator=self._gen)
            for k in range(int(hp["nminibatches"])):
                idx = perm[k * mb:(k + 1) * mb]
                if graphed:
                    sg["idx"].copy_(idx)
                    sg["graph"].replay()
                else:
                    acc += self._minibatch_step({key_: v[idx] for key_, v in batch.items()}, cliprange)
        if graphed:
            acc = sg["acc"].clone()
        steps = int(hp["noptepochs"]) * int(hp["nminibatches"])
        self.actor.load_policy(self.policy)
        self.updates += 1
        return {k: float(v) / steps for k, v in zip(STAT_KEYS, acc.tolist())}

    def learn(self, total_timesteps, callback=None, log=None):
        from . import distributed as fd
        while self.num_timesteps < total_timesteps:
            batch = self.collect()
            stats = self.update(batch)
            summary = fd.gather_success(self.vec, self.group)
            info = dict(stats, timesteps=self.num_timesteps, update=self.updates, episodes=summary["episodes"],
                        level=None if self.curriculum is None else self.curriculum.level)
            if summary["episodes"] > 0:
                info["success"] = dict(summary["success"])
                info["control_variation"] = summary["control_variation"]["all"]
            if self.curriculum is not None:
                info["level"] = self.curriculum.update(self.vec, summary)
                if self._rollout_kw["graph"] and self.vec.spec_index != self._spec_at_capture:
                    self.rollout = FusedRollout(self.vec, self.actor, self.n_steps, **self._rollout_kw)
                    self._spec_at_capture = self.vec.spec_index
            self.history.append(info)
            if log is not None:
                log(info)
            if callback is not None and callback(self, info) is False:
                break
        return self

    def deterministic_policy(self):
        st = self.actor.get_stats()
        dev = self._torch_dev
        mean = torch.as_tensor(st["obs_mean"], dtype=torch.float32, device=dev)
        std = torch.sqrt(torch.as_tensor(st["obs_var"], dtype=torch.float32, device=dev) + 1e-8)
        pi = self.policy.pi

        @torch.no_grad()
        def act(obs):
            x = torch.as_tensor(obs, dtype=torch.float32, device=dev)
            return pi(((x.reshape(x.shape[0], -1) - mean) / std).clamp(-10.0, 10.0))
        return act

    def save(self, path):
        st = self.actor.get_stats()
        sd = {k: v.detach().cpu().numpy() for k, v in self.policy.state_dict().items()}
        np.savez(path, **sd, **{"stat_" + k: np.asarray(v) for k, v in st.items()})

    def load(self, path):
        z = np.load(path)
        self.policy.load_state_dict({k: torch.as_tensor(z[k]) for k in z.files if not k.startswith("stat_")})
        self.actor.load_policy(self.policy)
        self.actor.set_stats(z["stat_obs_mean"], z["stat_obs_var"], float(z["stat_obs_count"]), float(z["stat_ret_mean"]),
                             float(z["stat_ret_var"]), float(z["stat_ret_count"]))
        return self
```

Baseline: 6.025 billion.

## Parallelize PPO learner kernels and make the HIP update path the default on GPU

The default update path changes from torch to the HIP learner on GPU. The learner is restructured: the advantage-moment kernel is split across many blocks per minibatch, and the gradient reduction becomes a two-stage grouped reduction. The grad-norm partials are produced as a by-product of that reduction. Adam apply runs across many blocks instead of one. The MMA helper is templated on K-blocks with independent accumulators, and the grad kernel stages network weights in LDS. Together these remove single-block serialization and repeated global reads, at the cost of extra launches and scratch buffers.

Result: no change. 6.018 billion, median of 6 (-0.1%).

```diff
diff --git a/fixed-wing-gym_amd/csrc/fwgym.hip b/fixed-wing-gym_amd/csrc/fwgym.hip
--- a/fixed-wing-gym_amd/csrc/fwgym.hip
+++ b/fixed-wing-gym_amd/csrc/fwgym.hip
@@ -1,6 +1,7 @@
 #include <math.h>
 #include <stdio.h>
 #include <string.h>
+#include <algorithm>
 #include <string>
 #include <vector>
 #include "fwgym_env.h"
@@ -2426,6 +2427,9 @@
     fwg_actor* head;
     PpoLayout L;
     float* d_slab;
+    float* d_part;
+    float* d_normp;
+    int* d_tstep;
     float* d_grad;
 };
 
@@ -2438,17 +2442,29 @@
     return b && b->obs && b->actions && b->values && b->logp && b->adv && b->returns;
 }
 static int ppo_launch_grad(fwg_learner* L, const fwg_ppo_batch* b, const int64_t* idx, int64_t mb, const float* moments,
-                           const float* params, const fwg_ppo_hparams* hp, float* grad_out, hipStream_t st) {
+                           const float* params, const fwg_ppo_hparams* hp, float* grad_out, const int32_t* step, hipStream_t st) {
     PpoGradArgs G;
     G.B = ppo_batch(b); G.idx = (const long long*)idx; G.mb = (long)mb; G.mom = moments; G.params = params;
     G.hp = (const PpoHparams*)hp; G.slab = L->d_slab; G.L = L->L;
     G.ntiles = (long)((mb + FWG_PPO_ROWS - 1) / FWG_PPO_ROWS);
     const unsigned nb = (unsigned)(G.ntiles < FWG_PPO_MAX_BLOCKS ? G.ntiles : FWG_PPO_MAX_BLOCKS);
-    hipLaunchKernelGGL(k_ppo_grad, dim3(nb), dim3(FWG_PPO_THREADS), (size_t)ppo_grad_lds_floats() * sizeof(float), st, G);
+    const int nk1 = (L->L.D + 15) / 16;
+    hipLaunchKernelGGL(k_ppo_grad, dim3(nb), dim3(FWG_PPO_THREADS), (size_t)ppo_grad_lds_floats(nk1) * sizeof(float), st, G);
     HIP_TRY(hipGetLastError());
-    const int n = L->L.P + FWG_PPO_NSTAT;
-    hipLaunchKernelGGL(k_ppo_reduce, dim3((unsigned)((n + FWG_PPO_THREADS - 1) / FWG_PPO_THREADS)), dim3(FWG_PPO_THREADS), 0, st,
-                       (const float*)L->d_slab, (int)nb, L->L, (const PpoHparams*)hp, grad_out);
+    const int ncb = ppo_ncb(L->L);
+    hipLaunchKernelGGL(k_ppo_reduce1, dim3((unsigned)(ncb * FWG_PPO_RGROUPS)), dim3(FWG_PPO_THREADS), 0, st, (const float*)L->d_slab, (int)nb,
+                       L->L, L->d_part);
+    HIP_TRY(hipGetLastError());
+    hipLaunchKernelGGL(k_ppo_reduce2, dim3((unsigned)ncb), dim3(FWG_PPO_THREADS), FWG_PPO_THREADS * sizeof(float), st, (const float*)L->d_part,
+                       L->L, (const PpoHparams*)hp, grad_out, L->d_normp, (const int*)step, L->d_tstep);
+    HIP_TRY(hipGetLastError());
+    return FWG_OK;
+}
+static int ppo_launch_apply(fwg_learner* L, const float* grad, int64_t mb, const fwg_ppo_hparams* hp, float* params, float* adam_m,
+                            float* adam_v, int32_t* step, float* stats_acc, hipStream_t st) {
+    hipLaunchKernelGGL(k_ppo_apply, dim3((unsigned)ppo_ncb(L->L)), dim3(FWG_PPO_APPLY_THREADS), FWG_PPO_APPLY_THREADS * sizeof(float), st,
+                       grad, (long)mb, L->L, (const PpoHparams*)hp, params, adam_m, adam_v, (int*)step, stats_acc, (const float*)L->d_normp,
+                       (const int*)L->d_tstep);
     HIP_TRY(hipGetLastError());
     return FWG_OK;
 }
@@ -2463,16 +2479,20 @@
     L->L = ppo_layout(head->D, head->act_dim);
     HIP_TRY(hipMalloc((void**)&L->d_slab, (size_t)FWG_PPO_MAX_BLOCKS * L->L.SW * sizeof(float)));
     HIP_TRY(hipMalloc((void**)&L->d_grad, (size_t)(L->L.P + FWG_PPO_NSTAT) * sizeof(float)));
+    HIP_TRY(hipMalloc((void**)&L->d_part, (size_t)FWG_PPO_RGROUPS * ppo_part_stride(L->L) * sizeof(float)));
+    HIP_TRY(hipMalloc((void**)&L->d_normp, (size_t)ppo_ncb(L->L) * sizeof(float)));
+    HIP_TRY(hipMalloc((void**)&L->d_tstep, sizeof(int)));
     HIP_TRY(hipMemset(L->d_slab, 0, (size_t)FWG_PPO_MAX_BLOCKS * L->L.SW * sizeof(float)));
     HIP_TRY(hipMemset(L->d_grad, 0, (size_t)(L->L.P + FWG_PPO_NSTAT) * sizeof(float)));
-    HIP_TRY(hipFuncSetAttribute((const void*)k_ppo_grad, hipFuncAttributeMaxDynamicSharedMemorySize, (int)(ppo_grad_lds_floats() * sizeof(float))));
+    HIP_TRY(hipFuncSetAttribute((const void*)k_ppo_grad, hipFuncAttributeMaxDynamicSharedMemorySize,
+                                (int)(ppo_grad_lds_floats((head->D + 15) / 16) * sizeof(float))));
     *out = L;
     return FWG_OK;
 }
 
 void fwg_learner_destroy(fwg_learner* L) {
     if (!L) return;
-    (void)hipFree(L->d_slab); (void)hipFree(L->d_grad);
+    (void)hipFree(L->d_slab); (void)hipFree(L->d_grad); (void)hipFree(L->d_part); (void)hipFree(L->d_normp); (void)hipFree(L->d_tstep);
     delete L;
 }
 
@@ -2481,8 +2501,23 @@
 int fwg_ppo_moments(fwg_learner* L, const float* adv, const int64_t* perm, int64_t mb, int n_minibatches, float* moments, void* stream) {
     if (!L || !adv || !perm || !moments) return fail_with(FWG_ERR_INVALID, "fwg_ppo_moments: null argument");
     if (mb < 1 || n_minibatches < 1) return fail_with(FWG_ERR_INVALID, "fwg_ppo_moments: mb and n_minibatches must be positive");
-    hipLaunchKernelGGL(k_ppo_moments, dim3((unsigned)n_minibatches), dim3(FWG_PPO_THREADS), FWG_PPO_THREADS * sizeof(double), (hipStream_t)stream,
-                       adv, (const long long*)perm, (long)mb, moments);
+    const int64_t cap = (int64_t)FWG_PPO_MAX_BLOCKS * L->L.SW / 4;
+    if ((int64_t)n_minibatches > cap) return fail_with(FWG_ERR_INVALID, "fwg_ppo_moments: too many minibatches");
+    int64_t nc = (1024 + n_minibatches - 1) / n_minibatches;
+    nc = std::min<int64_t>(nc, std::max<int64_t>(1, mb / 1024));
+    nc = std::max<int64_t>(1, std::min<int64_t>(nc, cap / n_minibatches));
+    double* part = reinterpret_cast<double*>(L->d_slab);
+    double* dev = part + cap;
+    const unsigned nblk = (unsigned)(n_minibatches * nc);
+    hipStream_t st = (hipStream_t)stream;
+    hipLaunchKernelGGL(k_ppo_mom_sum, dim3(nblk), dim3(FWG_PPO_THREADS), FWG_PPO_THREADS * sizeof(double), st, adv, (const long long*)perm,
+                       (long)mb, (int)nc, part);
+    HIP_TRY(hipGetLastError());
+    hipLaunchKernelGGL(k_ppo_mom_dev, dim3(nblk), dim3(FWG_PPO_THREADS), FWG_PPO_THREADS * sizeof(double), st, adv, (const long long*)perm,
+                       (long)mb, (int)nc, (const double*)part, dev);
+    HIP_TRY(hipGetLastError());
+    hipLaunchKernelGGL(k_ppo_mom_fin, dim3((unsigned)((n_minibatches + FWG_PPO_THREADS - 1) / FWG_PPO_THREADS)), dim3(FWG_PPO_THREADS), 0, st,
+                       (const double*)part, (const double*)dev, (long)mb, (int)nc, n_minibatches, moments);
     HIP_TRY(hipGetLastError());
     return FWG_OK;
 }
@@ -2491,17 +2526,17 @@
                  const fwg_ppo_hparams* hp, float* grad_out, void* stream) {
     if (!L || !ppo_batch_ok(b) || !idx || !moments || !params || !hp || !grad_out) return fail_with(FWG_ERR_INVALID, "fwg_ppo_grad: null argument");
     if (mb < 1) return fail_with(FWG_ERR_INVALID, "fwg_ppo_grad: mb must be positive");
-    return ppo_launch_grad(L, b, idx, mb, moments, params, hp, grad_out, (hipStream_t)stream);
+    return ppo_launch_grad(L, b, idx, mb, moments, params, hp, grad_out, nullptr, (hipStream_t)stream);
 }
 
 int fwg_ppo_apply(fwg_learner* L, const float* grad, int64_t mb, const fwg_ppo_hparams* hp, float* params, float* adam_m, float* adam_v,
                   int32_t* step, float* stats_acc, void* stream) {
     if (!L || !grad || !hp || !params || !adam_m || !adam_v || !step || !stats_acc) return fail_with(FWG_ERR_INVALID, "fwg_ppo_apply: null argument");
     if (mb < 1) return fail_with(FWG_ERR_INVALID, "fwg_ppo_apply: mb must be positive");
-    hipLaunchKernelGGL(k_ppo_apply, dim3(1), dim3(FWG_PPO_APPLY_THREADS), FWG_PPO_APPLY_THREADS * sizeof(float), (hipStream_t)stream,
-                       grad, (long)mb, L->L, (const PpoHparams*)hp, params, adam_m, adam_v, (int*)step, stats_acc);
+    hipLaunchKernelGGL(k_ppo_norm, dim3((unsigned)ppo_ncb(L->L)), dim3(FWG_PPO_THREADS), FWG_PPO_THREADS * sizeof(float), (hipStream_t)stream,
+                       grad, L->L, L->d_normp, (const int*)step, L->d_tstep);
     HIP_TRY(hipGetLastError());
-    return FWG_OK;
+    return ppo_launch_apply(L, grad, mb, hp, params, adam_m, adam_v, step, stats_acc, (hipStream_t)stream);
 }
 
 int fwg_ppo_step(fwg_learner* L, const fwg_ppo_batch* b, const int64_t* idx, int64_t mb, const float* moments, const fwg_ppo_hparams* hp,
@@ -2509,9 +2544,9 @@
     if (!L || !ppo_batch_ok(b) || !idx || !moments || !hp || !params || !adam_m || !adam_v || !step || !stats_acc)
         return fail_with(FWG_ERR_INVALID, "fwg_ppo_step: null argument");
     if (mb < 1) return fail_with(FWG_ERR_INVALID, "fwg_ppo_step: mb must be positive");
-    const int rc = ppo_launch_grad(L, b, idx, mb, moments, params, hp, L->d_grad, (hipStream_t)stream);
+    const int rc = ppo_launch_grad(L, b, idx, mb, moments, params, hp, L->d_grad, step, (hipStream_t)stream);
     if (rc != FWG_OK) return rc;
-    return fwg_ppo_apply(L, L->d_grad, mb, hp, params, adam_m, adam_v, step, stats_acc, stream);
+    return ppo_launch_apply(L, L->d_grad, mb, hp, params, adam_m, adam_v, step, stats_acc, (hipStream_t)stream);
 }
 
 int fwg_actor_pack(fwg_learner* L, const float* params, void* stream) {
diff --git a/fixed-wing-gym_amd/csrc/fwgym_learner.h b/fixed-wing-gym_amd/csrc/fwgym_learner.h
--- a/fixed-wing-gym_amd/csrc/fwgym_learner.h
+++ b/fixed-wing-gym_amd/csrc/fwgym_learner.h
@@ -33,57 +33,97 @@
 
 __device__ __forceinline__ float ppo_tanh(float z) { return tanh_prescaled(FWG_ACT_PRESCALE * z); }
 
-__device__ __forceinline__ void ppo_mma_tile(f32x16& acc, const float* A, int sam, int sak, int m0, int ml, const float* B, int sbk,
-                                             int sbn, int n0, int nl, int K, int kl, int l) {
+template <int NKB>
+__device__ __forceinline__ void ppo_mma(f32x16& acc, const float* A, int sam, int sak, int m0, const float* B, int sbk, int sbn, int n0, int l) {
     const int i = l & 31, half = l >> 5;
-    const bool mok = m0 + i < ml, nok = n0 + i < nl;
-    for (int k0 = 0; k0 < K; k0 += 16) {
+    frag_t ah[NKB], al[NKB], bh[NKB], bl[NKB];
+#pragma unroll
+    for (int kb = 0; kb < NKB; ++kb) {
         float a[8], b[8];
 #pragma unroll
         for (int t = 0; t < 8; ++t) {
-            const int k = k0 + 8 * half + t;
-            a[t] = (mok && k < kl) ? A[(m0 + i) * sam + k * sak] : 0.f;
-            b[t] = (nok && k < kl) ? B[k * sbk + (n0 + i) * sbn] : 0.f;
-        }
-        frag_t ah, al, bh, bl;
-        split8(a, ah, al);
-        split8(b, bh, bl);
-        acc = mma3<3>(ah, al, bh, bl, acc);
-    }
+            const int k = 16 * kb + 8 * half + t;
+            a[t] = A[(m0 + i) * sam + k * sak];
+            b[t] = B[k * sbk + (n0 + i) * sbn];
+        }
+        split8(a, ah[kb], al[kb]);
+        split8(b, bh[kb], bl[kb]);
+    }
+    if (NKB == 1) {
+        f32x16 ca = {0.f}, cb = {0.f};
+        mma3s<3>(ah[0], al[0], bh[0], bl[0], acc, ca, cb);
+#pragma unroll
+        for (int r = 0; r < 16; ++r) acc[r] += ca[r] + cb[r];
+        return;
+    }
+    f32x16 c[NKB];
+    c[0] = acc;
+#pragma unroll
+    for (int kb = 1; kb < NKB; ++kb)
+#pragma unroll
+        for (int r = 0; r < 16; ++r) c[kb][r] = 0.f;
+#pragma unroll
+    for (int kb = 0; kb < NKB; ++kb) c[kb] = fwg_mfma_bf16(al[kb], bh[kb], c[kb]);
+#pragma unroll
+    for (int kb = 0; kb < NKB; ++kb) c[kb] = fwg_mfma_bf16(ah[kb], bl[kb], c[kb]);
+#pragma unroll
+    for (int kb = 0; kb < NKB; ++kb) c[kb] = fwg_mfma_bf16(ah[kb], bh[kb], c[kb]);
+#pragma unroll
+    for (int kb = 1; kb < NKB; ++kb)
+#pragma unroll
+        for (int r = 0; r < 16; ++r) c[0][r] += c[kb][r];
+    acc = c[0];
 }
 __device__ __forceinline__ int ppo_acc_row(int r, int half) { return (r & 3) + 8 * (r >> 2) + 4 * half; }
 
-__global__ __launch_bounds__(FWG_PPO_THREADS) void k_ppo_moments(const float* __restrict__ adv, const long long* __restrict__ perm,
-                                                                 long mb, float* __restrict__ mom) {
-    extern __shared__ __attribute__((aligned(16))) float lds[];
-    double* red = reinterpret_cast<double*>(lds);
+__device__ __forceinline__ double ppo_block_sum_d(double v, double* red) {
     const int tid = threadIdx.x;
-    const long long* idx = perm + (long)blockIdx.x * mb;
-    double s = 0.0;
-    for (long i = tid; i < mb; i += FWG_PPO_THREADS) s += (double)adv[idx[i]];
-    red[tid] = s;
+    red[tid] = v;
     __syncthreads();
     for (int w = FWG_PPO_THREADS / 2; w > 0; w >>= 1) {
         if (tid < w) red[tid] += red[tid + w];
         __syncthreads();
     }
-    const double mean = red[0] / (double)mb;
+    const double s = red[0];
     __syncthreads();
+    return s;
+}
+__global__ __launch_bounds__(FWG_PPO_THREADS) void k_ppo_mom_sum(const float* __restrict__ adv, const long long* __restrict__ perm, long mb,
+                                                                 int nc, double* __restrict__ part) {
+    extern __shared__ __attribute__((aligned(16))) float lds[];
+    const long k = blockIdx.x / nc, c = blockIdx.x % nc;
+    const long long* idx = perm + k * mb;
+    const long i0 = c * mb / nc, i1 = (c + 1) * mb / nc;
+    double s = 0.0;
+    for (long i = i0 + threadIdx.x; i < i1; i += FWG_PPO_THREADS) s += (double)adv[idx[i]];
+    s = ppo_block_sum_d(s, reinterpret_cast<double*>(lds));
+    if (threadIdx.x == 0) part[blockIdx.x] = s;
+}
+__global__ __launch_bounds__(FWG_PPO_THREADS) void k_ppo_mom_dev(const float* __restrict__ adv, const long long* __restrict__ perm, long mb,
+                                                                 int nc, const double* __restrict__ part, double* __restrict__ dev) {
+    extern __shared__ __attribute__((aligned(16))) float lds[];
+    const long k = blockIdx.x / nc, c = blockIdx.x % nc;
+    const long long* idx = perm + k * mb;
+    const long i0 = c * mb / nc, i1 = (c + 1) * mb / nc;
+    double sum = 0.0;
+    for (int j = 0; j < nc; ++j) sum += part[k * nc + j];
+    const double mean = sum / (double)mb;
     double q = 0.0;
-    for (long i = tid; i < mb; i += FWG_PPO_THREADS) {
+    for (long i = i0 + threadIdx.x; i < i1; i += FWG_PPO_THREADS) {
         const double d = (double)adv[idx[i]] - mean;
         q += d * d;
     }
-    red[tid] = q;
-    __syncthreads();
-    for (int w = FWG_PPO_THREADS / 2; w > 0; w >>= 1) {
-        if (tid < w) red[tid] += red[tid + w];
-        __syncthreads();
-    }
-    if (tid == 0) {
-        mom[2 * blockIdx.x] = (float)mean;
-        mom[2 * blockIdx.x + 1] = (float)sqrt(red[0] / (double)mb) + 1e-8f;
-    }
+    q = ppo_block_sum_d(q, reinterpret_cast<double*>(lds));
+    if (threadIdx.x == 0) dev[blockIdx.x] = q;
+}
+__global__ __launch_bounds__(FWG_PPO_THREADS) void k_ppo_mom_fin(const double* __restrict__ part, const double* __restrict__ dev, long mb, int nc,
+                                                                 int nmb, float* __restrict__ mom) {
+    const int k = blockIdx.x * FWG_PPO_THREADS + threadIdx.x;
+    if (k >= nmb) return;
+    double s = 0.0, q = 0.0;
+    for (int j = 0; j < nc; ++j) { s += part[(long)k * nc + j]; q += dev[(long)k * nc + j]; }
+    mom[2 * k] = (float)(s / (double)mb);
+    mom[2 * k + 1] = (float)sqrt(q / (double)mb) + 1e-8f;
 }
 
 struct PpoGradArgs {
@@ -97,14 +137,33 @@
     float* slab;
     PpoLayout L;
 };
-__host__ __device__ inline int ppo_grad_lds_floats() { return 5 * FWG_PPO_ROWS * FWG_PPO_LS + 4 * FWG_PPO_ROWS + 8 * FWG_PPO_ROWS + 8 * FWG_PPO_ROWS; }
+__host__ __device__ inline int ppo_w1_stride(int nk1) { return 16 * nk1 + 1; }
+__host__ __device__ inline int ppo_net_lds_floats(int nk1) { return 64 * ppo_w1_stride(nk1) + 64 * FWG_PPO_LS + 4 * 64 + 64 + 64 + 4; }
+__host__ __device__ inline int ppo_grad_lds_floats(int nk1) {
+    return 5 * FWG_PPO_ROWS * FWG_PPO_LS + 4 * FWG_PPO_ROWS + 8 * FWG_PPO_ROWS + 8 * FWG_PPO_ROWS + 2 * ppo_net_lds_floats(nk1);
+}
+
+struct PpoRowRegs { float x[FWG_ACT_MAX_OBS / 4]; float s0, s1; };
+__device__ __forceinline__ void ppo_gather(const PpoGradArgs& G, long r0, float adv_mean, float adv_std, PpoRowRegs& R) {
+    const int tid = threadIdx.x, r = tid >> 2, q = tid & 3, D = G.L.D, A = G.L.A;
+    const bool ok = r0 + r < G.mb;
+    const long long row = ok ? G.idx[r0 + r] : 0;
+#pragma unroll
+    for (int i = 0; i < FWG_ACT_MAX_OBS / 4; ++i) {
+        const int f = q + 4 * i;
+        R.x[i] = (ok && f < D) ? G.B.obs[row * D + f] : 0.f;
+    }
+    R.s0 = (ok && q < A) ? G.B.act[row * A + q] : 0.f;
+    R.s1 = 0.f;
+    if (ok) R.s1 = q == 0 ? G.B.val[row] : q == 1 ? G.B.logp[row] : q == 2 ? (G.B.adv[row] - adv_mean) / adv_std : G.B.ret[row];
+}
 
 __global__ __launch_bounds__(FWG_PPO_THREADS) void k_ppo_grad(const PpoGradArgs G) {
     extern __shared__ __attribute__((aligned(16))) float lds[];
     constexpr int LS = FWG_PPO_LS;
     const int tid = threadIdx.x, l = tid & 63, wv = tid >> 6, half = l >> 5;
     const PpoLayout& L = G.L;
-    const int D = L.D, A = L.A, nk1 = (D + 15) / 16;
+    const int D = L.D, A = L.A, nk1 = (D + 15) / 16, W1S = ppo_w1_stride(nk1), NWF = ppo_net_lds_floats(nk1);
     float* Xs = lds;
     float* H1 = Xs + FWG_PPO_ROWS * LS;
     float* H2 = H1 + FWG_PPO_ROWS * LS;
@@ -113,67 +172,101 @@
     float* dO = Tb + FWG_PPO_ROWS * LS;
     float* rowf = dO + 4 * FWG_PPO_ROWS;
     float* red = rowf + 8 * FWG_PPO_ROWS;
+    float* Wn = red + 8 * FWG_PPO_ROWS;
     const PpoHparams hp = *G.hp;
     const float adv_mean = G.mom[0], adv_std = G.mom[1];
     const float inv_mb = 1.f / (float)G.mb, clip = (float)hp.cliprange, vf_coef = (float)hp.vf_coef;
     const float* P = G.params;
     const long t0 = (long)blockIdx.x * G.ntiles / gridDim.x, t1 = (long)(blockIdx.x + 1) * G.ntiles / gridDim.x;
     const int tm0 = 32 * (wv & 1), tn0 = 32 * (wv >> 1);
-    const int vo = tid >> 6, vk = tid & 63;
-    f32x16 gw1[2], gw2[2];
-#pragma unroll
-    for (int r = 0; r < 16; ++r) { gw1[0][r] = 0.f; gw1[1][r] = 0.f; gw2[0][r] = 0.f; gw2[1][r] = 0.f; }
-    float gw3[2] = {0.f, 0.f}, gb3[2] = {0.f, 0.f}, gb2[2] = {0.f, 0.f}, gb1[2] = {0.f, 0.f};
+    const int rr = tid >> 2, rq = tid & 3;
+    const int ck = tid & 63, cq = tid >> 6;
+    float* S = G.slab + (size_t)blockIdx.x * L.SW;
     float gls[FWG_ACT_MAX_ACT] = {0.f, 0.f, 0.f, 0.f}, st[FWG_PPO_NSTAT] = {0.f, 0.f, 0.f, 0.f};
-    for (long t = t0; t < t1; ++t) {
-        const long r0 = t * FWG_PPO_ROWS;
-        const int nrows = (int)(G.mb - r0 < FWG_PPO_ROWS ? G.mb - r0 : FWG_PPO_ROWS);
-        {
-            const int r = tid >> 2, q = tid & 3;
-            const bool ok = r < nrows;
-            const long long row = ok ? G.idx[r0 + r] : 0;
-            for (int f = 16 * q; f < 16 * q + 16; ++f) Xs[r * LS + f] = (ok && f < D) ? G.B.obs[row * D + f] : 0.f;
-            if (q == 0) {
-#pragma unroll
-                for (int a = 0; a < FWG_ACT_MAX_ACT; ++a) rowf[r * 8 + a] = (ok && a < A) ? G.B.act[row * A + a] : 0.f;
-                rowf[r * 8 + 4] = ok ? G.B.val[row] : 0.f;
-                rowf[r * 8 + 5] = ok ? G.B.logp[row] : 0.f;
-                rowf[r * 8 + 6] = ok ? (G.B.adv[row] - adv_mean) / adv_std : 0.f;
-                rowf[r * 8 + 7] = ok ? G.B.ret[row] : 0.f;
-            }
-        }
-        __syncthreads();
-#pragma unroll
-        for (int net = 0; net < 2; ++net) {
-            const int nout = net ? 1 : A;
-            const float *W1 = P + L.w1[net], *b1 = P + L.b1[net], *W2 = P + L.w2[net], *b2 = P + L.b2[net];
-            const float *W3 = P + L.w3[net], *b3 = P + L.b3[net];
+    PpoRowRegs R;
+    if (t0 < t1) ppo_gather(G, t0 * FWG_PPO_ROWS, adv_mean, adv_std, R);
+    for (int net = 0; net < 2; ++net) {
+        const int nout = net ? 1 : A;
+        float* W = Wn + net * NWF;
+        for (int e = tid; e < 64 * W1S; e += FWG_PPO_THREADS) {
+            const int n = e / W1S, k = e - n * W1S;
+            W[e] = k < D ? P[L.w1[net] + n * D + k] : 0.f;
+        }
+        W += 64 * W1S;
+        for (int e = tid; e < 64 * 64; e += FWG_PPO_THREADS) W[(e >> 6) * LS + (e & 63)] = P[L.w2[net] + e];
+        W += 64 * LS;
+        for (int e = tid; e < 4 * 64; e += FWG_PPO_THREADS) W[e] = (e >> 6) < nout ? P[L.w3[net] + e] : 0.f;
+        W += 4 * 64;
+        if (tid < 64) { W[tid] = P[L.b1[net] + tid]; W[64 + tid] = P[L.b2[net] + tid]; }
+        if (tid < 4) W[128 + tid] = tid < nout ? P[L.b3[net] + tid] : 0.f;
+    }
+#pragma unroll 1
+    for (int net = 0; net < 2; ++net) {
+        const int nout = net ? 1 : A;
+        const float* W1 = Wn + net * NWF;
+        const float* W2 = W1 + 64 * W1S;
+        const float* W3 = W2 + 64 * LS;
+        const float* b1 = W3 + 4 * 64;
+        const float* b2 = b1 + 64;
+        const float* b3 = b2 + 64;
+        const int n = tn0 + (l & 31);
+        f32x16 gw1 = {0.f}, gw2 = {0.f};
+        float gw3p[FWG_ACT_MAX_ACT] = {0.f, 0.f, 0.f, 0.f}, gb3p[FWG_ACT_MAX_ACT] = {0.f, 0.f, 0.f, 0.f}, gb2p = 0.f, gb1p = 0.f;
+        if (net == 1 && t0 < t1) ppo_gather(G, t0 * FWG_PPO_ROWS, adv_mean, adv_std, R);
+        for (long t = t0; t < t1; ++t) {
+            const long r0 = t * FWG_PPO_ROWS;
+            const int nrows = (int)(G.mb - r0 < FWG_PPO_ROWS ? G.mb - r0 : FWG_PPO_ROWS);
+#pragma unroll
+            for (int i = 0; i < FWG_ACT_MAX_OBS / 4; ++i) Xs[rr * LS + rq + 4 * i] = R.x[i];
+            rowf[rr * 8 + rq] = R.s0;
+            rowf[rr * 8 + 4 + rq] = R.s1;
+            if (t + 1 < t1) ppo_gather(G, r0 + FWG_PPO_ROWS, adv_mean, adv_std, R);
+            __syncthreads();
+            f32x16 h1v;
             {
                 f32x16 acc = {0.f};
-                ppo_mma_tile(acc, Xs, LS, 1, tm0, 64, W1, 1, D, tn0, 64, 16 * nk1, D, l);
-                const int n = tn0 + (l & 31);
+                switch (nk1) {
+                    case 1: ppo_mma<1>(acc, Xs, LS, 1, tm0, W1, 1, W1S, tn0, l); break;
+                    case 2: ppo_mma<2>(acc, Xs, LS, 1, tm0, W1, 1, W1S, tn0, l); break;
+                    case 3: ppo_mma<3>(acc, Xs, LS, 1, tm0, W1, 1, W1S, tn0, l); break;
+                    default: ppo_mma<4>(acc, Xs, LS, 1, tm0, W1, 1, W1S, tn0, l); break;
+                }
                 const float bn = b1[n];
 #pragma unroll
-                for (int r = 0; r < 16; ++r) H1[(tm0 + ppo_acc_row(r, half)) * LS + n] = ppo_tanh(acc[r] + bn);
+                for (int r = 0; r < 16; ++r) {
+                    h1v[r] = ppo_tanh(acc[r] + bn);
+                    H1[(tm0 + ppo_acc_row(r, half)) * LS + n] = h1v[r];
+                }
             }
             __syncthreads();
             {
                 f32x16 acc = {0.f};
-                ppo_mma_tile(acc, H1, LS, 1, tm0, 64, W2, 1, 64, tn0, 64, 64, 64, l);
-                const int n = tn0 + (l & 31);
+                ppo_mma<4>(acc, H1, LS, 1, tm0, W2, 1, LS, tn0, l);
                 const float bn = b2[n];
 #pragma unroll
                 for (int r = 0; r < 16; ++r) H2[(tm0 + ppo_acc_row(r, half)) * LS + n] = ppo_tanh(acc[r] + bn);
             }
             __syncthreads();
-            if (vo < nout) {
-                float o = b3[vo];
-                for (int k = 0; k < 64; ++k) o += H2[vk * LS + k] * W3[vo * 64 + k];
-                dO[vk * 4 + vo] = o;
-            }
-            __syncthreads();
-            if (tid < FWG_PPO_ROWS) {
-                const int r = tid;
+            {
+                float o[FWG_ACT_MAX_ACT];
+#pragma unroll
+                for (int a = 0; a < FWG_ACT_MAX_ACT; ++a) o[a] = 0.f;
+#pragma unroll
+                for (int k = 16 * rq; k < 16 * rq + 16; ++k) {
+                    const float h = H2[rr * LS + k];
+#pragma unroll
+                    for (int a = 0; a < FWG_ACT_MAX_ACT; ++a)
+                        if (a < nout) o[a] += h * W3[a * 64 + k];
+                }
+#pragma unroll
+                for (int a = 0; a < FWG_ACT_MAX_ACT; ++a) {
+                    if (a < nout) {
+                        o[a] += __shfl_xor(o[a], 1, 64);
+                        o[a] += __shfl_xor(o[a], 2, 64);
+                        o[a] += b3[a];
+                    }
+                }
+                const int r = rr;
                 const bool ok = r < nrows;
                 const float* rf = rowf + r * 8;
                 if (net == 0) {
@@ -184,7 +277,7 @@
                         if (a < A) {
                             const float s = P[L.ls + a];
                             is[a] = expf(-s);
-                            z[a] = (rf[a] - dO[r * 4 + a]) * is[a];
+                            z[a] = (rf[a] - o[a]) * is[a];
                             nl += 0.5f * z[a] * z[a] + s;
                         }
                     }
@@ -194,89 +287,101 @@
                     const float g1 = -adv, g2 = (ratio >= 1.f - clip && ratio <= 1.f + clip) ? -adv : 0.f;
                     const float dr = p1 > p2 ? g1 : (p1 < p2 ? g2 : 0.5f * (g1 + g2));
                     const float gn = ok ? -ratio * dr * inv_mb : 0.f;
-#pragma unroll
-                    for (int a = 0; a < FWG_ACT_MAX_ACT; ++a) {
-                        dO[r * 4 + a] = a < A ? -gn * z[a] * is[a] : 0.f;
-                        gls[a] += a < A ? gn * (1.f - z[a] * z[a]) : 0.f;
-                    }
-                    if (ok) {
-                        const float kl = nl + rf[5];
-                        st[0] += fmaxf(p1, p2);
-                        st[2] += 0.5f * kl * kl;
-                        st[3] += fabsf(ratio - 1.f) > clip ? 1.f : 0.f;
+                    if (rq == 0) {
+#pragma unroll
+                        for (int a = 0; a < FWG_ACT_MAX_ACT; ++a) {
+                            dO[r * 4 + a] = a < A ? -gn * z[a] * is[a] : 0.f;
+                            gls[a] += a < A ? gn * (1.f - z[a] * z[a]) : 0.f;
+                        }
+                        if (ok) {
+                            const float kl = nl + rf[5];
+                            st[0] += fmaxf(p1, p2);
+                            st[2] += 0.5f * kl * kl;
+                            st[3] += fabsf(ratio - 1.f) > clip ? 1.f : 0.f;
+                        }
                     }
                 } else {
-                    const float v = dO[r * 4], ov = rf[4], R = rf[7], d = v - ov;
+                    const float v = o[0], ov = rf[4], ret = rf[7], d = v - ov;
                     const float vc = ov + fminf(fmaxf(d, -clip), clip);
-                    const float l1 = (v - R) * (v - R), l2 = (vc - R) * (vc - R);
-                    const float g1 = 2.f * (v - R), g2 = (d >= -clip && d <= clip) ? 2.f * (vc - R) : 0.f;
+                    const float l1 = (v - ret) * (v - ret), l2 = (vc - ret) * (vc - ret);
+                    const float g1 = 2.f * (v - ret), g2 = (d >= -clip && d <= clip) ? 2.f * (vc - ret) : 0.f;
                     const float dv = l1 > l2 ? g1 : (l1 < l2 ? g2 : 0.5f * (g1 + g2));
-                    dO[r * 4] = ok ? vf_coef * 0.5f * dv * inv_mb : 0.f;
-                    if (ok) st[1] += 0.5f * fmaxf(l1, l2);
+                    if (rq == 0) {
+                        dO[r * 4] = ok ? vf_coef * 0.5f * dv * inv_mb : 0.f;
+                        if (ok) st[1] += 0.5f * fmaxf(l1, l2);
+                    }
                 }
             }
             __syncthreads();
-            if (vo < nout) {
-                float s = 0.f, sb = 0.f;
-                for (int r = 0; r < FWG_PPO_ROWS; ++r) { s += dO[r * 4 + vo] * H2[r * LS + vk]; sb += dO[r * 4 + vo]; }
-                gw3[net] += s;
-                if (vk == 0) gb3[net] += sb;
-            }
-            for (int j = 0; j < FWG_PPO_ROWS * 64 / FWG_PPO_THREADS; ++j) {
-                const int e = tid + FWG_PPO_THREADS * j, r = e >> 6, k = e & 63;
+            for (int j = 0; j < FWG_PPO_ROWS / 4; ++j) {
+                const int r = cq + 4 * j;
+                const float h = H2[r * LS + ck];
                 float s = 0.f;
-                for (int o = 0; o < nout; ++o) s += dO[r * 4 + o] * W3[o * 64 + k];
-                const float h = H2[r * LS + k];
-                Gb[r * LS + k] = s * (1.f - h * h);
+#pragma unroll
+                for (int o = 0; o < FWG_ACT_MAX_ACT; ++o) {
+                    if (o < nout) {
+                        const float d = dO[r * 4 + o];
+                        s += d * W3[o * 64 + ck];
+                        gw3p[o] += d * h;
+                        gb3p[o] += d;
+                    }
+                }
+                const float g = s * (1.f - h * h);
+                Gb[r * LS + ck] = g;
+                gb2p += g;
             }
             __syncthreads();
             {
                 f32x16 acc = {0.f};
-                ppo_mma_tile(acc, Gb, LS, 1, tm0, 64, W2, 64, 1, tn0, 64, 64, 64, l);
-                const int n = tn0 + (l & 31);
+                ppo_mma<4>(acc, Gb, LS, 1, tm0, W2, LS, 1, tn0, l);
 #pragma unroll
                 for (int r = 0; r < 16; ++r) {
-                    const int m = tm0 + ppo_acc_row(r, half);
-                    const float h = H1[m * LS + n];
-                    Tb[m * LS + n] = acc[r] * (1.f - h * h);
-                }
-                ppo_mma_tile(gw2[net], Gb, 1, LS, tm0, 64, H1, LS, 1, tn0, 64, 64, 64, l);
-                if (tid < 64) {
-                    float s = 0.f;
-                    for (int r = 0; r < FWG_PPO_ROWS; ++r) s += Gb[r * LS + tid];
-                    gb2[net] += s;
-                }
+                    const float g = acc[r] * (1.f - h1v[r] * h1v[r]);
+                    Tb[(tm0 + ppo_acc_row(r, half)) * LS + n] = g;
+                    gb1p += g;
+                }
+                ppo_mma<4>(gw2, Gb, 1, LS, tm0, H1, LS, 1, tn0, l);
             }
             __syncthreads();
-            if (tn0 < D) ppo_mma_tile(gw1[net], Tb, 1, LS, tm0, 64, Xs, LS, 1, tn0, D, 64, 64, l);
-            if (tid < 64) {
-                float s = 0.f;
-                for (int r = 0; r < FWG_PPO_ROWS; ++r) s += Tb[r * LS + tid];
-                gb1[net] += s;
-            }
-            __syncthreads();
-        }
-    }
-    float* S = G.slab + (size_t)blockIdx.x * L.SW;
-#pragma unroll
-    for (int net = 0; net < 2; ++net) {
-        const int nout = net ? 1 : A;
-        const int n = tn0 + (l & 31);
+            if (tn0 < D) ppo_mma<4>(gw1, Tb, 1, LS, tm0, Xs, LS, 1, tn0, l);
+            __syncthreads();
+        }
+        float* sc_w3 = H1;
+        float* sc_b2 = sc_w3 + 4 * 4 * 64;
+        float* sc_b1 = sc_b2 + 4 * 64;
+        float* sc_b3 = sc_b1 + 4 * 64;
+#pragma unroll
+        for (int o = 0; o < FWG_ACT_MAX_ACT; ++o) {
+            sc_w3[(o * 4 + cq) * 64 + ck] = gw3p[o];
+            if (ck == 0) sc_b3[o * 4 + cq] = gb3p[o];
+        }
+        sc_b2[cq * 64 + ck] = gb2p;
+        sc_b1[wv * 64 + l] = gb1p;
 #pragma unroll
         for (int r = 0; r < 16; ++r) {
             const int m = tm0 + ppo_acc_row(r, half);
-            if (n < D) S[L.w1[net] + m * D + n] = gw1[net][r];
-            S[L.w2[net] + m * 64 + n] = gw2[net][r];
-        }
-        if (vo < nout) {
-            S[L.w3[net] + vo * 64 + vk] = gw3[net];
-            if (vk == 0) S[L.b3[net] + vo] = gb3[net];
-        }
-        if (tid < 64) { S[L.b1[net] + tid] = gb1[net]; S[L.b2[net] + tid] = gb2[net]; }
-    }
-    if (tid < FWG_PPO_ROWS) {
-#pragma unroll
-        for (int a = 0; a < 4; ++a) { red[tid * 8 + a] = gls[a]; red[tid * 8 + 4 + a] = st[a]; }
+            if (n < D) S[L.w1[net] + m * D + n] = gw1[r];
+            S[L.w2[net] + m * 64 + n] = gw2[r];
+        }
+        __syncthreads();
+        if (cq < nout) {
+            const float* p = sc_w3 + cq * 4 * 64 + ck;
+            S[L.w3[net] + cq * 64 + ck] = ((p[0] + p[64]) + p[128]) + p[192];
+            if (ck == 0) {
+                const float* b = sc_b3 + cq * 4;
+                S[L.b3[net] + cq] = ((b[0] + b[1]) + b[2]) + b[3];
+            }
+        }
+        if (tid < 64) {
+            const float* p = sc_b2 + tid;
+            S[L.b2[net] + tid] = ((p[0] + p[64]) + p[128]) + p[192];
+            const float* q = sc_b1 + 2 * (tid >> 5) * 64 + (tid & 31);
+            S[L.b1[net] + tid] = ((q[0] + q[32]) + q[64]) + q[96];
+        }
+    }
+    if (rq == 0) {
+#pragma unroll
+        for (int a = 0; a < 4; ++a) { red[rr * 8 + a] = gls[a]; red[rr * 8 + 4 + a] = st[a]; }
     }
     __syncthreads();
     if (tid < 8) {
@@ -287,41 +392,83 @@
     }
 }
 
-__global__ __launch_bounds__(FWG_PPO_THREADS) void k_ppo_reduce(const float* __restrict__ slab, int nslab, const PpoLayout L,
-                                                                const PpoHparams* __restrict__ hp, float* __restrict__ grad) {
+#define FWG_PPO_RGROUPS 16
+__host__ __device__ inline int ppo_ncb(const PpoLayout& L) { return (L.P + FWG_PPO_NSTAT + FWG_PPO_THREADS - 1) / FWG_PPO_THREADS; }
+__host__ __device__ inline int ppo_part_stride(const PpoLayout& L) { return ppo_ncb(L) * FWG_PPO_THREADS; }
+
+__global__ __launch_bounds__(FWG_PPO_THREADS) void k_ppo_reduce1(const float* __restrict__ slab, int nslab, const PpoLayout L,
+                                                                 float* __restrict__ part) {
+    const int ncb = ppo_ncb(L), g = blockIdx.x / ncb, cb = blockIdx.x % ncb;
+    const int j = cb * FWG_PPO_THREADS + threadIdx.x;
+    if (j >= L.P + FWG_PPO_NSTAT) return;
+    const int b0 = g * nslab / FWG_PPO_RGROUPS, b1 = (g + 1) * nslab / FWG_PPO_RGROUPS;
+    float s = 0.f;
+    for (int b = b0; b < b1; ++b) s += slab[(size_t)b * L.SW + j];
+    part[(size_t)g * ppo_part_stride(L) + j] = s;
+}
+__device__ __forceinline__ float ppo_block_sum_f(float v, float* red) {
+    const int tid = threadIdx.x;
+    red[tid] = v;
+    __syncthreads();
+    for (int w = FWG_PPO_THREADS / 2; w > 0; w >>= 1) {
+        if (tid < w) red[tid] += red[tid + w];
+        __syncthreads();
+    }
+    return red[0];
+}
+__global__ __launch_bounds__(FWG_PPO_THREADS) void k_ppo_reduce2(const float* __restrict__ part, const PpoLayout L, const PpoHparams* __restrict__ hp,
+                                                                 float* __restrict__ grad, float* __restrict__ normp, const int* __restrict__ step,
+                                                                 int* __restrict__ tstep) {
+    extern __shared__ __attribute__((aligned(16))) float lds[];
     const int j = blockIdx.x * FWG_PPO_THREADS + threadIdx.x;
-    if (j >= L.P + FWG_PPO_NSTAT) return;
     float s = 0.f;
-    for (int b = 0; b < nslab; ++b) s += slab[(size_t)b * L.SW + j];
-    if (j >= L.ls && j < L.ls + L.A) s -= (float)hp->ent_coef;
-    grad[j] = s;
+    if (j < L.P + FWG_PPO_NSTAT) {
+#pragma unroll
+        for (int g = 0; g < FWG_PPO_RGROUPS; ++g) s += part[(size_t)g * ppo_part_stride(L) + j];
+        if (j >= L.ls && j < L.ls + L.A) s -= (float)hp->ent_coef;
+        grad[j] = s;
+    }
+    const float sq = ppo_block_sum_f(j < L.P ? s * s : 0.f, lds);
+    if (threadIdx.x == 0) {
+        normp[blockIdx.x] = sq;
+        if (step != nullptr && blockIdx.x == 0) tstep[0] = *step + 1;
+    }
+}
+__global__ __launch_bounds__(FWG_PPO_THREADS) void k_ppo_norm(const float* __restrict__ grad, const PpoLayout L, float* __restrict__ normp,
+                                                              const int* __restrict__ step, int* __restrict__ tstep) {
+    extern __shared__ __attribute__((aligned(16))) float lds[];
+    const int j = blockIdx.x * FWG_PPO_THREADS + threadIdx.x;
+    const float g = j < L.P ? grad[j] : 0.f;
+    const float sq = ppo_block_sum_f(g * g, lds);
+    if (threadIdx.x == 0) {
+        normp[blockIdx.x] = sq;
+        if (blockIdx.x == 0) tstep[0] = *step + 1;
+    }
 }
 
 __global__ __launch_bounds__(FWG_PPO_APPLY_THREADS) void k_ppo_apply(const float* __restrict__ grad, long mb, const PpoLayout L,
                                                                      const PpoHparams* __restrict__ hp, float* __restrict__ params,
                                                                      float* __restrict__ m1, float* __restrict__ m2, int* __restrict__ step,
-                                                                     float* __restrict__ acc) {
+                                                                     float* __restrict__ acc, const float* __restrict__ normp,
+                                                                     const int* __restrict__ tstep) {
     extern __shared__ __attribute__((aligned(16))) float lds[];
-    const int tid = threadIdx.x;
+    const int tid = threadIdx.x, ncb = ppo_ncb(L);
+    for (int c = tid; c < ncb; c += FWG_PPO_APPLY_THREADS) lds[c] = normp[c];
     float ent = 0.f;
-    if (tid == 0)
+    if (blockIdx.x == 0 && tid == 0)
         for (int a = 0; a < L.A; ++a) ent += params[L.ls + a] + 1.4189385332046727f;
+    __syncthreads();
     float ss = 0.f;
-    for (int j = tid; j < L.P; j += FWG_PPO_APPLY_THREADS) ss += grad[j] * grad[j];
-    lds[tid] = ss;
-    __syncthreads();
-    for (int w = FWG_PPO_APPLY_THREADS / 2; w > 0; w >>= 1) {
-        if (tid < w) lds[tid] += lds[tid + w];
-        __syncthreads();
-    }
+    for (int c = 0; c < ncb; ++c) ss += lds[c];
     const PpoHparams h = *hp;
-    const float norm = sqrtf(lds[0]);
+    const float norm = sqrtf(ss);
     const float coef = fminf((float)h.max_grad_norm / (norm + 1e-6f), 1.f);
-    const int t = *step + 1;
+    const int t = *tstep;
     const double bc1 = 1.0 - pow(h.beta1, (double)t), bc2 = 1.0 - pow(h.beta2, (double)t);
     const float step_size = (float)(h.lr / bc1), bc2_sqrt = (float)sqrt(bc2);
     const float b2 = (float)h.beta2, w1 = (float)(1.0 - h.beta1), w2 = (float)(1.0 - h.beta2), eps = (float)h.eps;
-    for (int j = tid; j < L.P; j += FWG_PPO_APPLY_THREADS) {
+    const int j = blockIdx.x * FWG_PPO_APPLY_THREADS + tid;
+    if (j < L.P) {
         const float g = grad[j] * coef;
         float m = m1[j], v = m2[j];
         m = m + w1 * (g - m);
@@ -329,8 +476,7 @@
         m1[j] = m; m2[j] = v;
         params[j] -= step_size * (m / (sqrtf(v) / bc2_sqrt + eps));
     }
-    __syncthreads();
-    if (tid == 0) {
+    if (blockIdx.x == 0 && tid == 0) {
         const float inv = 1.f / (float)mb;
         *step = t;
         acc[0] += grad[L.P] * inv;
@@ -340,6 +486,7 @@
         acc[4] += grad[L.P + 3] * inv;
     }
 }
+
 
 __global__ __launch_bounds__(256) void k_actor_pack(const float* __restrict__ params, const PpoLayout L, int nk1, frag_t* __restrict__ frags,
                                                     float* __restrict__ bias, float* __restrict__ log_std) {
diff --git a/fixed-wing-gym_amd/gym_fixed_wing/ppo.py b/fixed-wing-gym_amd/gym_fixed_wing/ppo.py
--- a/fixed-wing-gym_amd/gym_fixed_wing/ppo.py
+++ b/fixed-wing-gym_amd/gym_fixed_wing/ppo.py
@@ -53,22 +53,29 @@
     return loss, stats
 
 
+def resolve_update(update, device):
+    if update == "auto":
+        return "hip" if torch.device(device).type == "cuda" else "torch"
+    return update
+
+
 class PPO(object):
 
     def __init__(self, vec, policy=None, seed=0, fused=None, graph=True, curriculum=None, group=None, precise=True,
-                 graph_update=True, update="torch", **kw):
+                 graph_update=True, update="auto", **kw):
         from .actor import DeviceActor
         hp = dict(PPO2_DEFAULTS)
         unknown = set(kw) - set(hp)
         if unknown:
             raise TypeError("unknown PPO hyper-parameters: {}".format(sorted(unknown)))
         hp.update(kw)
-        if update not in ("torch", "hip"):
-            raise ValueError("update must be 'torch' or 'hip', not {!r}".format(update))
-        self.update_path = update
+        if update not in ("auto", "torch", "hip"):
+            raise ValueError("update must be 'auto', 'torch' or 'hip', not {!r}".format(update))
         self.hp, self.vec, self.group = hp, vec, group
         self.n_steps = int(hp["n_steps"])
         self._torch_dev = getattr(vec._mem, "device", torch.device("cpu"))
+        update = resolve_update(update, self._torch_dev)
+        self.update_path = update
         torch.manual_seed(seed)
         self.policy = (sb_init_(MlpPolicy(vec.obs_dim)) if policy is None else policy).to(self._torch_dev)
         self.actor = DeviceActor.for_env(vec, seed=seed, gamma=hp["gamma"], precise=precise)
```
